# dselivanov/rsparse

Hardware: AMD Instinct MI355X
Metric: als_iterations_per_sec (higher is better)
Workload: dtype f32 (Gram products of rows > 512 / <= 32 non-zeros as 2 x fp16 / 3 x bf16 split terms of the fp32 operands, fp32 accumulate; everything else fp32); 1 GPU; WRMF implicit ALS, CG(3), synthetic 10000000x1000000, 500155883 nnz, rank 128, lambda 0.1; survey_config=3, feedback=implicit, n_items=1000000, nnz=500155883, rank=128, solver=conjugate_gradient, cg_steps=3, parallelism=rows sharded x1, factors replicated

## Files before the change

include/rsparse_wrmf_hip.h:

```cpp
#ifndef RSPARSE_WRMF_HIP_H
#define RSPARSE_WRMF_HIP_H

#include <stddef.h>
#include <stdint.h>

#ifdef __cplusplus
extern "C" {
#endif

#define RSPARSE_HIP_OK 0
#define RSPARSE_HIP_ERR_INVALID 1
#define RSPARSE_HIP_ERR_UNSUPPORTED 2
#define RSPARSE_HIP_ERR_RUNTIME 3
#define RSPARSE_HIP_ERR_NUMERIC 4

#define RSPARSE_SOLVER_CHOLESKY 0
#define RSPARSE_SOLVER_CONJUGATE_GRADIENT 1
#define RSPARSE_SOLVER_NNLS 2

#define RSPARSE_HIP_MAX_RANK 256
#define RSPARSE_HIP_MAX_RANK_F64 128

const char* rsparse_hip_last_error(void);
int rsparse_hip_abi_version(void);
int rsparse_hip_device_count(void);
int rsparse_hip_set_device(int device);


int rsparse_hip_als_implicit_float(int n_rows, int n_cols, const int32_t* col_ptrs,
                                   const int32_t* row_indices, const double* values,
                                   const float* X, float* Y, const float* XtX, int rank,
                                   double lambda, int n_threads, unsigned solver,
                                   unsigned cg_steps, int with_biases, int is_x_bias_last_row,
                                   double global_bias, float* global_bias_base, int global_bias_base_len,
                                   int initialize_bias_base, double* loss_out);

int rsparse_hip_als_implicit_double(int n_rows, int n_cols, const int32_t* col_ptrs,
                                    const int32_t* row_indices, const double* values,
                                    const double* X, double* Y, const double* XtX, int rank,
                                    double lambda, int n_threads, unsigned solver,
                                    unsigned cg_steps, int with_biases, int is_x_bias_last_row,
                                    double global_bias, double* global_bias_base, int global_bias_base_len,
                                    int initialize_bias_base, double* loss_out);

int rsparse_hip_als_explicit_float(int n_rows, int n_cols, const int32_t* col_ptrs,
                                   const int32_t* row_indices, const double* values,
                                   const float* X, float* Y, const float* cnt_X, int rank,
                                   double lambda, unsigned n_threads, unsigned solver,
                                   unsigned cg_steps, int dynamic_lambda, int with_biases,
                                   int is_x_bias_last_row, double* loss_out);

int rsparse_hip_als_explicit_double(int n_rows, int n_cols, const int32_t* col_ptrs,
                                    const int32_t* row_indices, const double* values,
                                    const double* X, double* Y, const double* cnt_X, int rank,
                                    double lambda, unsigned n_threads, unsigned solver,
                                    unsigned cg_steps, int dynamic_lambda, int with_biases,
                                    int is_x_bias_last_row, double* loss_out);

int rsparse_hip_gramian_float(const float* X, int rank, int64_t n, double lambda, float* XtX_out);
int rsparse_hip_gramian_double(const double* X, int rank, int64_t n, double lambda, double* XtX_out);

int rsparse_hip_initialize_biases_float(int n_users, int n_items, const int32_t* csc_p, const int32_t* csc_i,
                                        double* csc_x, const int32_t* csr_p, const int32_t* csr_i, double* csr_x,
                                        float* user_bias, float* item_bias, double lambda, int dynamic_lambda,
                                        int non_negative, int calculate_global_bias, int is_explicit_feedback,
                                        double* global_bias_out);
int rsparse_hip_initialize_biases_double(int n_users, int n_items, const int32_t* csc_p, const int32_t* csc_i,
                                         double* csc_x, const int32_t* csr_p, const int32_t* csr_i, double* csr_x,
                                         double* user_bias, double* item_bias, double lambda, int dynamic_lambda,
                                         int non_negative, int calculate_global_bias, int is_explicit_feedback,
                                         double* global_bias_out);


typedef struct rsparse_hip_csc rsparse_hip_csc;

int rsparse_hip_csc_create_host(int n_rows, int n_cols, const int32_t* col_ptrs,
                                const int32_t* row_indices, const double* values,
                                rsparse_hip_csc** out);
int rsparse_hip_csc_create_device(int n_rows, int n_cols, const int32_t* d_col_ptrs,
                                  const int32_t* d_row_indices, const float* d_values,
                                  rsparse_hip_csc** out);
int rsparse_hip_csc_destroy(rsparse_hip_csc* m);

int rsparse_hip_csc_transpose_device(int n_rows, int n_cols, const int32_t* d_p, const int32_t* d_i,
                                     const float* d_x, int32_t* d_pt, int32_t* d_it, float* d_xt, void* stream);
int rsparse_hip_values_to_float_device(int64_t n, const double* d_src, float* d_dst, void* stream);
int rsparse_hip_csc_freeze_values(rsparse_hip_csc* m, int frozen);

int rsparse_hip_csc_info(const rsparse_hip_csc* m, int64_t info_out[40]);

int rsparse_hip_gramian_device(const float* d_X, int rank, int64_t n, double lambda,
                               float* d_XtX_out, double* d_sumsq_out, void* stream);

int rsparse_hip_gramian_absmax_device(const float* d_X, int rank, int64_t n, double lambda, float* d_XtX_out,
                                      double* d_sumsq_out, float* d_absmax_inout, void* stream);

int rsparse_hip_als_implicit_device(const rsparse_hip_csc* conf, const float* d_X, float* d_Y,
                                    const float* d_XtX, int rank, double lambda, unsigned solver,
                                    unsigned cg_steps, const float* d_absmax, double* d_loss_rows_out, void* stream);

int rsparse_hip_als_explicit_device(const rsparse_hip_csc* conf, const float* d_X, float* d_Y,
                                    int rank, double lambda, unsigned solver, unsigned cg_steps,
                                    int dynamic_lambda, double* d_loss_rows_out, void* stream);

int rsparse_hip_als_implicit_bias_device(const rsparse_hip_csc* conf, const float* d_X, float* d_Y,
                                         const float* d_XtX, int rank, double lambda, unsigned solver,
                                         int is_x_bias_last_row, double* d_loss_rows_out, void* stream);

int rsparse_hip_als_implicit_global_bias_device(const rsparse_hip_csc* conf, const float* d_X, float* d_Y,
                                                const float* d_XtX, int rank, double lambda, unsigned solver,
                                                unsigned cg_steps, int with_biases, int is_x_bias_last_row,
                                                double global_bias, int double_threshold, const float* d_absmax,
                                                double* d_loss_rows_out, void* stream);

int rsparse_hip_initialize_biases_implicit_device(const rsparse_hip_csc* c_ui, const rsparse_hip_csc* c_iu,
                                                  float* d_user_bias, float* d_item_bias, double lambda,
                                                  int non_negative, int calculate_global_bias,
                                                  double* global_bias_out, void* stream);

int rsparse_hip_als_explicit_bias_device(const rsparse_hip_csc* conf, const float* d_X, float* d_Y, int rank,
                                         double lambda, unsigned solver, unsigned cg_steps, int dynamic_lambda,
                                         int is_x_bias_last_row, double* d_loss_rows_out, void* stream);

int rsparse_hip_values_subtract_mean_device(int64_t n, float* d_x, float* d_x_other, double* mean_out, void* stream);

int rsparse_hip_initialize_biases_explicit_device(rsparse_hip_csc* c_ui, rsparse_hip_csc* c_iu, float* d_user_bias,
                                                  float* d_item_bias, double lambda, int dynamic_lambda,
                                                  int non_negative, int calculate_global_bias,
                                                  double* global_bias_out, void* stream);

int rsparse_hip_bias_sweep_explicit_device(const rsparse_hip_csc* conf, const float* d_other_bias, double lambda,
                                           int dynamic_lambda, int non_negative, float* d_out, void* stream);
int rsparse_hip_bias_prep_implicit_device(const rsparse_hip_csc* conf, int n_other, double lambda, double* d_means,
                                          double* d_adj, void* stream);
int rsparse_hip_bias_sweep_implicit_device(const rsparse_hip_csc* conf, const float* d_other_bias, int n_other,
                                           const double* d_other_sum, const double* d_means, const double* d_adj,
                                           int non_negative, double global_bias, float* d_out, void* stream);

int rsparse_hip_weighted_sumsq_device(const float* d_X, int rank, int64_t n, const float* d_w,
                                      double* d_out, void* stream);


#define RSPARSE_HIP_NA_INTEGER INT32_MIN
#define RSPARSE_HIP_MAX_TOPK 256
#define RSPARSE_HIP_MAX_TOPK_LARGE 8192

int rsparse_hip_top_product(const double* x, const double* y, int nr, int nc, int rank, unsigned k,
                            unsigned n_threads, const int32_t* not_recommend_p,
                            const int32_t* not_recommend_j, const int32_t* exclude, int n_exclude,
                            double glob_mean, int32_t* res, double* scores);

int rsparse_hip_top_product_device(const float* d_U, const float* d_V, int n_users, int n_items, int rank,
                                   int k, const int32_t* d_not_recommend_p, const int32_t* d_not_recommend_j,
                                   const int32_t* d_exclude0, int n_exclude, double glob_mean,
                                   int32_t* d_res, float* d_scores, void* stream);

int rsparse_hip_top_product_f64_device(const float* d_U, const float* d_V, const double* d_U64, const double* d_V64,
                                       int n_users, int n_items, int rank, int k, int extra,
                                       const int32_t* d_not_recommend_p, const int32_t* d_not_recommend_j,
                                       const int32_t* d_exclude0, int n_exclude, double glob_mean, int32_t* d_res,
                                       double* d_scores, void* stream);

int rsparse_hip_top_candidates_device(const float* d_U, const float* d_V, int n_users, int n_items, int rank, int k,
                                      const int32_t* d_cand_p, const int32_t* d_cand_j, const int32_t* d_not_recommend_p,
                                      const int32_t* d_not_recommend_j, const int32_t* d_exclude0, int n_exclude,
                                      double glob_mean, int32_t* d_res, double* d_scores, void* stream);
int rsparse_hip_top_candidates_f64_device(const double* d_U, const double* d_V, int n_users, int n_items, int rank, int k,
                                          const int32_t* d_cand_p, const int32_t* d_cand_j, const int32_t* d_not_recommend_p,
                                          const int32_t* d_not_recommend_j, const int32_t* d_exclude0, int n_exclude,
                                          double glob_mean, int32_t* d_res, double* d_scores, void* stream);
int rsparse_hip_top_candidates(const double* x, const double* y, int nr, int nc, int rank, unsigned k, unsigned n_threads,
                               const int32_t* cand_p, const int32_t* cand_j, const int32_t* not_recommend_p,
                               const int32_t* not_recommend_j, const int32_t* exclude, int n_exclude, double glob_mean,
                               int32_t* res, double* scores);


int rsparse_hip_normalize_items_device(const float* d_V, int n_items, int ld, int c0, int c1, float* d_Vn32, double* d_Vn64,
                                       int32_t* d_flags, void* stream);
int rsparse_hip_normalize_items_f64_device(const double* d_V, int n_items, int ld, int c0, int c1, float* d_Vn32,
                                           double* d_Vn64, int32_t* d_flags, void* stream);

int rsparse_hip_similar_items_device(const float* d_Vn32, const double* d_Vn64, int n_items, int r, const int32_t* d_query,
                                     int n_q, int k, int exclude_self, const int32_t* d_exclude0, int n_exclude,
                                     int32_t* d_res, double* d_scores, void* stream);

int rsparse_hip_similar_items(const double* components, int rank, int n_items, int first_row, int n_rows, const int32_t* query,
                              int n_q, int k, int exclude_self, const int32_t* exclude, int n_exclude, int32_t* res,
                              double* scores);


int rsparse_hip_ranking_metrics(const int32_t* predictions, int n_users, int k, const int32_t* actual_p,
                                const int32_t* actual_j, const double* actual_x, double* ap_out, double* ndcg_out);

int rsparse_hip_ranking_metrics_device(const int32_t* d_predictions, int n_users, int k, const int32_t* d_actual_p,
                                       const int32_t* d_actual_j, const double* d_actual_x, double* d_ap_out,
                                       double* d_ndcg_out, void* stream);


#define RSPARSE_HIP_MAX_CUTOFFS 16
int rsparse_hip_hit_metrics_device(const int32_t* d_predictions, int n_users, int k, const int32_t* d_actual_p,
                                   const int32_t* d_actual_j, const int32_t* cutoffs, int n_cutoffs, int32_t* d_hits,
                                   int32_t* d_first, double* d_precision, double* d_recall, double* d_hit, double* d_mrr,
                                   int32_t* d_first_seen, int n_items, void* stream);

int rsparse_hip_hit_metrics(const int32_t* predictions, int n_users, int k, const int32_t* actual_p, const int32_t* actual_j,
                            const int32_t* cutoffs, int n_cutoffs, int32_t* hits, int32_t* first, double* precision,
                            double* recall, double* hit, double* mrr, int32_t* first_seen, int n_items);


int rsparse_hip_list_metrics_device(const int32_t* d_predictions, int n_users, int k, const int32_t* cutoffs, int n_cutoffs,
                                    const int32_t* d_item_count, const int64_t* d_item_info, int n_items, int32_t* d_valid,
                                    int64_t* d_count_sum, int64_t* d_info_sum, double* d_popularity, double* d_novelty,
                                    int32_t* d_exposure, void* stream);

int rsparse_hip_list_metrics(const int32_t* predictions, int n_users, int k, const int32_t* cutoffs, int n_cutoffs,
                             const int32_t* item_count, const int64_t* item_info, int n_items, int32_t* valid,
                             int64_t* count_sum, int64_t* info_sum, double* popularity, double* novelty, int32_t* exposure);

int rsparse_hip_item_inv_norms_device(const float* d_V, int n_items, int ld, int c0, int c1, double* d_inv, void* stream);
int rsparse_hip_item_inv_norms_f64_device(const double* d_V, int n_items, int ld, int c0, int c1, double* d_inv, void* stream);

int rsparse_hip_list_diversity_device(const int32_t* d_predictions, int n_users, int k, const int32_t* cutoffs, int n_cutoffs,
                                      const float* d_V, int n_items, int ld, int c0, int c1, const double* d_inv,
                                      int32_t* d_counted, double* d_diversity, void* stream);
int rsparse_hip_list_diversity_f64_device(const int32_t* d_predictions, int n_users, int k, const int32_t* cutoffs,
                                          int n_cutoffs, const double* d_V, int n_items, int ld, int c0, int c1,
                                          const double* d_inv, int32_t* d_counted, double* d_diversity, void* stream);

int rsparse_hip_list_diversity(const int32_t* predictions, int n_users, int k, const int32_t* cutoffs, int n_cutoffs,
                               const float* V, int n_items, int ld, int c0, int c1, int32_t* counted, double* diversity);
int rsparse_hip_list_diversity_f64(const int32_t* predictions, int n_users, int k, const int32_t* cutoffs, int n_cutoffs,
                                   const double* V, int n_items, int ld, int c0, int c1, int32_t* counted, double* diversity);


int rsparse_hip_mmr_rerank_device(const int32_t* d_lists, const double* d_scores, int n_users, int n_pool, int k, double trade_off,
                                  const float* d_V, int n_items, int ld, int c0, int c1, const double* d_inv, int32_t* d_items,
                                  double* d_scores_out, int32_t* d_positions, double* d_objective, void* stream);
int rsparse_hip_mmr_rerank_f64_device(const int32_t* d_lists, const double* d_scores, int n_users, int n_pool, int k,
                                      double trade_off, const double* d_V, int n_items, int ld, int c0, int c1, const double* d_inv,
                                      int32_t* d_items, double* d_scores_out, int32_t* d_positions, double* d_objective,
                                      void* stream);

// ... 179 lines not shown
```

rsparse_amd/_lib.py:

```python
import ctypes
from pathlib import Path

import os

LIB_PATH = Path(os.environ.get("RSPARSE_HIP_LIB", Path(__file__).resolve().parent / "lib" / "librsparse_wrmf_hip.so"))

OK, ERR_INVALID, ERR_UNSUPPORTED, ERR_RUNTIME, ERR_NUMERIC = 0, 1, 2, 3, 4
SOLVER_CHOLESKY, SOLVER_CG, SOLVER_NNLS = 0, 1, 2
MAX_NEGATIVES = 8192
MAX_CUTOFFS = 16
RANKS_BATCH = 1024

_c_int, _c_uint, _c_dbl, _c_i64, _c_u64 = ctypes.c_int, ctypes.c_uint, ctypes.c_double, ctypes.c_int64, ctypes.c_uint64
_vp = ctypes.c_void_p

SIGNATURES = {
    "rsparse_hip_last_error": (ctypes.c_char_p, []),
    "rsparse_hip_abi_version": (_c_int, []),
    "rsparse_hip_device_count": (_c_int, []),
    "rsparse_hip_set_device": (_c_int, [_c_int]),
    "rsparse_hip_als_implicit_float": (_c_int, [_c_int, _c_int, _vp, _vp, _vp, _vp, _vp, _vp, _c_int, _c_dbl, _c_int,
                                                _c_uint, _c_uint, _c_int, _c_int, _c_dbl, _vp, _c_int, _c_int, _vp]),
    "rsparse_hip_als_implicit_double": (_c_int, [_c_int, _c_int, _vp, _vp, _vp, _vp, _vp, _vp, _c_int, _c_dbl, _c_int,
                                                 _c_uint, _c_uint, _c_int, _c_int, _c_dbl, _vp, _c_int, _c_int, _vp]),
    "rsparse_hip_als_explicit_float": (_c_int, [_c_int, _c_int, _vp, _vp, _vp, _vp, _vp, _vp, _c_int, _c_dbl, _c_uint,
                                                _c_uint, _c_uint, _c_int, _c_int, _c_int, _vp]),
    "rsparse_hip_als_explicit_double": (_c_int, [_c_int, _c_int, _vp, _vp, _vp, _vp, _vp, _vp, _c_int, _c_dbl, _c_uint,
                                                 _c_uint, _c_uint, _c_int, _c_int, _c_int, _vp]),
    "rsparse_hip_gramian_float": (_c_int, [_vp, _c_int, _c_i64, _c_dbl, _vp]),
    "rsparse_hip_gramian_double": (_c_int, [_vp, _c_int, _c_i64, _c_dbl, _vp]),
    "rsparse_hip_csc_create_host": (_c_int, [_c_int, _c_int, _vp, _vp, _vp, ctypes.POINTER(_vp)]),
    "rsparse_hip_csc_create_device": (_c_int, [_c_int, _c_int, _vp, _vp, _vp, ctypes.POINTER(_vp)]),
    "rsparse_hip_gramian_absmax_device": (_c_int, [_vp, _c_int, _c_i64, _c_dbl, _vp, _vp, _vp, _vp]),
    "rsparse_hip_csc_destroy": (_c_int, [_vp]),
    "rsparse_hip_csc_info": (_c_int, [_vp, ctypes.POINTER(_c_i64)]),
    "rsparse_hip_csc_freeze_values": (_c_int, [_vp, _c_int]),
    "rsparse_hip_als_implicit_bias_device": (_c_int, [_vp, _vp, _vp, _vp, _c_int, _c_dbl, _c_uint, _c_int, _vp, _vp]),
    "rsparse_hip_als_implicit_global_bias_device": (_c_int, [_vp, _vp, _vp, _vp, _c_int, _c_dbl, _c_uint, _c_uint, _c_int,
                                                             _c_int, _c_dbl, _c_int, _vp, _vp, _vp]),
    "rsparse_hip_initialize_biases_implicit_device": (_c_int, [_vp, _vp, _vp, _vp, _c_dbl, _c_int, _c_int,
                                                               ctypes.POINTER(_c_dbl), _vp]),
    "rsparse_hip_initialize_biases_float": (_c_int, [_c_int, _c_int, _vp, _vp, _vp, _vp, _vp, _vp, _vp, _vp, _c_dbl, _c_int,
                                                     _c_int, _c_int, _c_int, ctypes.POINTER(_c_dbl)]),
    "rsparse_hip_initialize_biases_double": (_c_int, [_c_int, _c_int, _vp, _vp, _vp, _vp, _vp, _vp, _vp, _vp, _c_dbl, _c_int,
                                                      _c_int, _c_int, _c_int, ctypes.POINTER(_c_dbl)]),
    "rsparse_hip_als_explicit_bias_device": (_c_int, [_vp, _vp, _vp, _c_int, _c_dbl, _c_uint, _c_uint, _c_int, _c_int,
                                                      _vp, _vp]),
    "rsparse_hip_initialize_biases_explicit_device": (_c_int, [_vp, _vp, _vp, _vp, _c_dbl, _c_int, _c_int, _c_int,
                                                               ctypes.POINTER(_c_dbl), _vp]),
    "rsparse_hip_values_subtract_mean_device": (_c_int, [_c_i64, _vp, _vp, ctypes.POINTER(_c_dbl), _vp]),
    "rsparse_hip_bias_sweep_explicit_device": (_c_int, [_vp, _vp, _c_dbl, _c_int, _c_int, _vp, _vp]),
    "rsparse_hip_bias_prep_implicit_device": (_c_int, [_vp, _c_int, _c_dbl, _vp, _vp, _vp]),
    "rsparse_hip_bias_sweep_implicit_device": (_c_int, [_vp, _vp, _c_int, _vp, _vp, _vp, _c_int, _c_dbl, _vp, _vp]),
    "rsparse_hip_bias_sweep_explicit_f64_device": (_c_int, [_vp, _vp, _c_dbl, _c_int, _c_int, _vp, _vp]),
    "rsparse_hip_bias_prep_implicit_f64_device": (_c_int, [_vp, _c_int, _c_dbl, _vp, _vp, _vp]),
    "rsparse_hip_bias_sweep_implicit_f64_device": (_c_int, [_vp, _vp, _c_int, _vp, _vp, _vp, _c_int, _c_dbl, _vp, _vp]),
    "rsparse_hip_csc_transpose_device": (_c_int, [_c_int, _c_int, _vp, _vp, _vp, _vp, _vp, _vp, _vp]),
    "rsparse_hip_values_to_float_device": (_c_int, [_c_i64, _vp, _vp, _vp]),
    "rsparse_hip_gramian_device": (_c_int, [_vp, _c_int, _c_i64, _c_dbl, _vp, _vp, _vp]),
    "rsparse_hip_als_implicit_device": (_c_int, [_vp, _vp, _vp, _vp, _c_int, _c_dbl, _c_uint, _c_uint, _vp, _vp, _vp]),
    "rsparse_hip_als_explicit_device": (_c_int, [_vp, _vp, _vp, _c_int, _c_dbl, _c_uint, _c_uint, _c_int, _vp, _vp]),
    "rsparse_hip_weighted_sumsq_device": (_c_int, [_vp, _c_int, _c_i64, _vp, _vp, _vp]),
    "rsparse_hip_top_product": (_c_int, [_vp, _vp, _c_int, _c_int, _c_int, _c_uint, _c_uint, _vp, _vp, _vp, _c_int, _c_dbl, _vp, _vp]),
    "rsparse_hip_top_product_device": (_c_int, [_vp, _vp, _c_int, _c_int, _c_int, _c_int, _vp, _vp, _vp, _c_int, _c_dbl, _vp, _vp, _vp]),
    "rsparse_hip_top_product_f64_device": (_c_int, [_vp, _vp, _vp, _vp, _c_int, _c_int, _c_int, _c_int, _c_int, _vp, _vp, _vp,
                                                    _c_int, _c_dbl, _vp, _vp, _vp]),
    "rsparse_hip_normalize_items_device": (_c_int, [_vp, _c_int, _c_int, _c_int, _c_int, _vp, _vp, _vp, _vp]),
    "rsparse_hip_normalize_items_f64_device": (_c_int, [_vp, _c_int, _c_int, _c_int, _c_int, _vp, _vp, _vp, _vp]),
    "rsparse_hip_similar_items_device": (_c_int, [_vp, _vp, _c_int, _c_int, _vp, _c_int, _c_int, _c_int, _vp, _c_int, _vp, _vp, _vp]),
    "rsparse_hip_similar_items": (_c_int, [_vp, _c_int, _c_int, _c_int, _c_int, _vp, _c_int, _c_int, _c_int, _vp, _c_int, _vp, _vp]),
    "rsparse_hip_ranking_metrics": (_c_int, [_vp, _c_int, _c_int, _vp, _vp, _vp, _vp, _vp]),
    "rsparse_hip_ranking_metrics_device": (_c_int, [_vp, _c_int, _c_int, _vp, _vp, _vp, _vp, _vp, _vp]),
    "rsparse_hip_hit_metrics_device": (_c_int, [_vp, _c_int, _c_int, _vp, _vp, _vp, _c_int, _vp, _vp, _vp, _vp, _vp, _vp, _vp, _c_int,
                                                _vp]),
    "rsparse_hip_hit_metrics": (_c_int, [_vp, _c_int, _c_int, _vp, _vp, _vp, _c_int, _vp, _vp, _vp, _vp, _vp, _vp, _vp, _c_int]),
    "rsparse_hip_list_metrics_device": (_c_int, [_vp, _c_int, _c_int, _vp, _c_int, _vp, _vp, _c_int, _vp, _vp, _vp, _vp, _vp, _vp, _vp]),
    "rsparse_hip_list_metrics": (_c_int, [_vp, _c_int, _c_int, _vp, _c_int, _vp, _vp, _c_int, _vp, _vp, _vp, _vp, _vp, _vp]),
    "rsparse_hip_item_inv_norms_device": (_c_int, [_vp, _c_int, _c_int, _c_int, _c_int, _vp, _vp]),
    "rsparse_hip_item_inv_norms_f64_device": (_c_int, [_vp, _c_int, _c_int, _c_int, _c_int, _vp, _vp]),
    "rsparse_hip_list_diversity_device": (_c_int, [_vp, _c_int, _c_int, _vp, _c_int, _vp, _c_int, _c_int, _c_int, _c_int, _vp, _vp, _vp,
                                                   _vp]),
    "rsparse_hip_list_diversity_f64_device": (_c_int, [_vp, _c_int, _c_int, _vp, _c_int, _vp, _c_int, _c_int, _c_int, _c_int, _vp, _vp,
                                                       _vp, _vp]),
    "rsparse_hip_list_diversity": (_c_int, [_vp, _c_int, _c_int, _vp, _c_int, _vp, _c_int, _c_int, _c_int, _c_int, _vp, _vp]),
    "rsparse_hip_list_diversity_f64": (_c_int, [_vp, _c_int, _c_int, _vp, _c_int, _vp, _c_int, _c_int, _c_int, _c_int, _vp, _vp]),
    "rsparse_hip_mmr_rerank_device": (_c_int, [_vp, _vp, _c_int, _c_int, _c_int, _c_dbl, _vp, _c_int, _c_int, _c_int, _c_int, _vp, _vp, _vp, _vp, _vp, _vp]),
    "rsparse_hip_mmr_rerank_f64_device": (_c_int, [_vp, _vp, _c_int, _c_int, _c_int, _c_dbl, _vp, _c_int, _c_int, _c_int, _c_int, _vp, _vp, _vp, _vp, _vp, _vp]),
    "rsparse_hip_mmr_rerank": (_c_int, [_vp, _vp, _c_int, _c_int, _c_int, _c_dbl, _vp, _c_int, _c_int, _c_int, _c_int, _vp, _vp, _vp, _vp]),
    "rsparse_hip_mmr_rerank_f64": (_c_int, [_vp, _vp, _c_int, _c_int, _c_int, _c_dbl, _vp, _c_int, _c_int, _c_int, _c_int, _vp, _vp, _vp, _vp]),
    "rsparse_hip_held_out_ranks_device": (_c_int, [_vp, _vp, _c_int, _c_int, _c_int, _vp, _vp, _vp, _c_int, _vp, _vp, _c_int, _vp, _vp,
                                                   _vp, _vp]),
    "rsparse_hip_rank_summary_device": (_c_int, [_c_int, _vp, _vp, _vp, _vp, _vp, _vp, _vp, _vp, _vp, _vp]),
    "rsparse_hip_held_out_ranks": (_c_int, [_vp, _vp, _c_int, _c_int, _c_int, _vp, _vp, _vp, _c_int, _vp, _vp, _vp, _vp, _vp, _vp, _vp,
                                            _vp, _vp, _vp]),
    "rsparse_hip_score_pairs_device": (_c_int, [_vp, _vp, _c_int, _c_int, _c_int, _vp, _vp, _c_dbl, _vp, _vp, _vp, _vp, _vp]),
    "rsparse_hip_score_pairs_f64_device": (_c_int, [_vp, _vp, _c_int, _c_int, _c_int, _vp, _vp, _c_dbl, _vp, _vp, _vp, _vp, _vp]),
    "rsparse_hip_top_candidates_device": (_c_int, [_vp, _vp, _c_int, _c_int, _c_int, _c_int, _vp, _vp, _vp, _vp, _vp, _c_int, _c_dbl, _vp,
                                                   _vp, _vp]),
    "rsparse_hip_top_candidates_f64_device": (_c_int, [_vp, _vp, _c_int, _c_int, _c_int, _c_int, _vp, _vp, _vp, _vp, _vp, _c_int, _c_dbl,
                                                       _vp, _vp, _vp]),
    "rsparse_hip_top_candidates": (_c_int, [_vp, _vp, _c_int, _c_int, _c_int, _c_uint, _c_uint, _vp, _vp, _vp, _vp, _vp, _c_int, _c_dbl,
                                            _vp, _vp]),
    "rsparse_hip_explain_device": (_c_int, [_vp, _c_int, _c_int, _vp, _c_dbl, _c_dbl, _c_int, _vp, _vp, _vp, _vp, _vp, _vp, _vp, _vp,
                                            _vp, _vp, _vp]),
    "rsparse_hip_explain_f64_device": (_c_int, [_vp, _c_int, _c_int, _vp, _c_dbl, _c_dbl, _c_int, _vp, _vp, _vp, _vp, _vp, _vp, _vp,
                                                _vp, _vp, _vp, _vp]),
    "rsparse_hip_init_factors_device": (_c_int, [_c_u64, _c_int, _c_i64, _c_int, _c_int, _c_i64, _c_dbl, _c_int, _c_int, _vp, _vp]),
    "rsparse_hip_init_factors_f64_device": (_c_int, [_c_u64, _c_int, _c_i64, _c_int, _c_int, _c_i64, _c_dbl, _c_int, _c_int, _vp,
                                                     _vp]),
    "rsparse_hip_sample_negatives_device": (_c_int, [_c_u64, _c_i64, _c_int, _c_int, _c_int, _vp, _vp, _vp, _vp, _vp, _vp, _c_i64, _vp]),
    "rsparse_hip_sample_negatives": (_c_int, [_c_u64, _c_i64, _c_int, _c_int, _c_int, _vp, _vp, _vp, _vp, _vp, _vp, _c_i64]),
    "rsparse_hip_weights_prefix_device": (_c_int, [_vp, _c_int, _vp, _vp]),
    "rsparse_hip_sample_negatives_weighted_device": (_c_int, [_c_u64, _c_i64, _c_int, _c_int, _c_int, _vp, _vp, _vp, _vp, _vp, _vp, _vp, _c_i64, _vp, _vp]),
    "rsparse_hip_sample_negatives_weighted": (_c_int, [_c_u64, _c_i64, _c_int, _c_int, _c_int, _vp, _vp, _vp, _vp, _vp, _vp, _vp, _c_i64, _vp]),
    "rsparse_hip_split_rows_device": (_c_int, [_c_u64, _c_i64, _c_int, _c_int, _c_u64, _c_int, _c_int, _vp, _vp, _vp, _c_int, _vp, _vp, _vp, _vp, _vp, _vp, _vp, _c_i64, _c_i64, _vp]),
    "rsparse_hip_split_rows": (_c_int, [_c_u64, _c_i64, _c_int, _c_int, _c_u64, _c_int, _c_int, _vp, _vp, _vp, _c_int, _vp, _vp, _vp, _vp, _vp, _vp, _vp, _c_i64, _c_i64]),
    "rsparse_hip_confidence_moments_device": (_c_int, [_c_int, _c_i64, _vp, _vp, _c_int, _vp, _vp, _vp]),
    "rsparse_hip_confidence_table_device": (_c_int, [_c_int, _c_int, _vp, _vp, _vp, _c_dbl, _c_dbl, _c_dbl, _vp, _vp]),
    "rsparse_hip_confidence_apply_device": (_c_int, [_c_int, _c_int, _c_i64, _vp, _vp, _vp, _vp, _vp, _c_int, _c_int, _c_dbl, _c_dbl, _vp, _c_int, _vp]),
    "rsparse_hip_confidence": (_c_int, [_c_int, _c_int, _c_int, _vp, _vp, _vp, _c_dbl, _c_dbl, _c_int, _c_int, _vp]),
    "rsparse_hip_events_to_csr_device": (_c_int, [_c_i64, _c_int, _c_int, _vp, _vp, _vp, _vp, _c_int, _c_dbl, _c_dbl, _c_int, _vp, _vp, _vp, _vp, _vp,
                                                  _c_i64, ctypes.POINTER(_c_i64), _vp]),
    "rsparse_hip_events_to_csr": (_c_int, [_c_i64, _c_int, _c_int, _vp, _vp, _vp, _vp, _c_int, _c_dbl, _c_dbl, _c_int, _vp, _vp, _vp, _vp, _vp,
                                           _c_i64, ctypes.POINTER(_c_i64)]),
    "rsparse_hip_sparse_approximation": (_c_int, [_c_int, _c_int, _vp, _vp, _c_int, _vp, _vp, _c_int, _vp]),
    "rsparse_hip_csc_f64_create_device": (_c_int, [_c_int, _c_int, _vp, _vp, _vp, ctypes.POINTER(_vp)]),
    "rsparse_hip_csc_f64_destroy": (_c_int, [_vp]),
    "rsparse_hip_gramian_f64_device": (_c_int, [_vp, _c_int, _c_i64, _c_dbl, _vp, _vp, _vp]),
    "rsparse_hip_als_f64_device": (_c_int, [_vp, _c_int, _vp, _vp, _vp, _c_int, _c_dbl, _c_uint, _c_uint, _c_int, _c_int,
                                            _c_int, _c_dbl, _vp, _vp]),
    "rsparse_hip_initialize_biases_f64_device": (_c_int, [_vp, _vp, _vp, _vp, _c_dbl, _c_int, _c_int, _c_int, _c_int,
                                                          ctypes.POINTER(_c_dbl), _vp]),
    "rsparse_hip_values_subtract_mean_f64_device": (_c_int, [_c_i64, _vp, _vp, ctypes.POINTER(_c_dbl), _vp]),
    "rsparse_hip_weighted_sumsq_f64_device": (_c_int, [_vp, _c_int, _c_i64, _vp, _vp, _vp]),
    "rsparse_hip_profile_enable": (_c_int, [_c_int]),
    "rsparse_hip_set_launch_mode": (_c_int, [_c_int]),
    "rsparse_hip_set_f64_long_rows": (_c_int, [_c_int, _c_int]),
    "rsparse_hip_profile_last": (_c_int, [ctypes.POINTER(_c_dbl)]),
    "rsparse_hip_profile_last_names": (_c_int, [ctypes.c_char_p, _c_int]),
    "rsparse_hip_take_numeric_failures": (_c_int, [ctypes.POINTER(_c_i64), ctypes.POINTER(_c_i64)]),
    "rsparse_hip_ctx_create": (_c_int, [_c_int, _vp, _c_int, ctypes.POINTER(_vp)]),
    "rsparse_hip_ctx_destroy": (_c_int, [_vp]),
    "rsparse_hip_ctx_set_matrix": (_c_int, [_vp, _c_int, _c_int, _vp, _vp, _vp, _vp, _vp, _vp, _c_int, _c_int]),
    "rsparse_hip_ctx_set_factors": (_c_int, [_vp, _c_int, _vp, _vp]),
    "rsparse_hip_ctx_get_factors": (_c_int, [_vp, _vp, _vp]),
    "rsparse_hip_ctx_half_iteration": (_c_int, [_vp, _c_int, _c_int, _c_dbl, _c_uint, _c_uint, _c_int, ctypes.POINTER(_c_dbl)]),
    "rsparse_hip_ctx_take_numeric_failures": (_c_int, [_vp, ctypes.POINTER(_c_i64), ctypes.POINTER(_c_i64)]),
    "rsparse_hip_ctx_info": (_c_int, [_vp, ctypes.POINTER(_c_i64), ctypes.POINTER(_c_dbl)]),
}


class RsparseHipError(RuntimeError):
    def __init__(self, code, msg):
        super().__init__("librsparse_wrmf_hip: [%d] %s" % (code, msg))
        self.code = code


class UnsupportedOnDevice(RsparseHipError, NotImplementedError):
    """RSPARSE_HIP_ERR_UNSUPPORTED: the reference-side shim would keep its CPU path here."""


_lib = None


def load():
    global _lib
    if _lib is None:
        if not LIB_PATH.exists():
            raise RuntimeError(
                "%s not found -- the HIP extension is required (no CPU fallback). "
                "Build it with `python -m rsparse_amd.build`." % LIB_PATH)
        try:
            import torch
            torch.cuda.is_available()
        except ImportError:
            pass
        lib = ctypes.CDLL(str(LIB_PATH))
        for name, (res, args) in SIGNATURES.items():
            f = getattr(lib, name)
            f.restype, f.argtypes = res, args
        _lib = lib
    return _lib


def check(code):
    if code == OK:
        return
    msg = load().rsparse_hip_last_error().decode("utf-8", "replace")
# ... 4 lines not shown
```

rsparse_amd/build.py:

```python
import subprocess
import sys
import time
from concurrent.futures import ThreadPoolExecutor
from pathlib import Path

PKG = Path(__file__).resolve().parent
CSRC = PKG / "csrc"
SRC = [CSRC / n for n in ("wrmf_kernels.hip", "wrmf_cgq.hip", "wrmf_cgp.hip", "wrmf_ne.hip", "wrmf_chol.hip", "wrmf_chol_wave.hip", "wrmf_chol_mf.hip", "wrmf_cg_mf.hip", "wrmf_chol_lr.hip",
                          "wrmf_topk.hip", "wrmf_topk_large.hip", "wrmf_similar.hip", "wrmf_metrics.hip", "wrmf_hits.hip", "wrmf_lists.hip", "wrmf_diversity.hip", "wrmf_mmr.hip", "wrmf_ranks.hip", "wrmf_score.hip", "wrmf_candidates.hip", "wrmf_sample.hip", "wrmf_sample_weighted.hip", "wrmf_split.hip", "wrmf_confidence.hip", "wrmf_events.hip", "wrmf_explain.hip", "wrmf_init.hip", "wrmf_ingest.hip", "wrmf_nnls.hip", "wrmf_bias.hip", "wrmf_lu.hip",
                          "wrmf_f64.hip", "wrmf_wide.hip", "wrmf_wide_cg.hip", "wrmf_ctx_kernels.hip", "wrmf_schedule.cpp", "wrmf_capi.cpp", "wrmf_f64_capi.cpp", "wrmf_ctx.cpp")]
HEADERS = [CSRC / "wrmf_chol_mf.attrs.csv", CSRC / "wrmf_mf.h", CSRC / "wrmf_internal.h", CSRC / "wrmf_capi_common.h", CSRC / "wrmf_schedule.h", CSRC / "wrmf_device.h", CSRC / "wrmf_sample_team.h", CSRC / "wrmf_wave.h", CSRC / "wrmf_ldlt.h", CSRC / "wrmf_f64.h", PKG.parent / "include" / "rsparse_wrmf_hip.h"]
DEPS = SRC + HEADERS
OUT = PKG / "lib" / "librsparse_wrmf_hip.so"
FLAGS = ["--offload-arch=gfx950", "-O3", "-std=c++17", "-fPIC"]


EXTRA_FLAGS = {n: ["-mllvm", "-forceattrs-csv-path=" + str(CSRC / "wrmf_chol_mf.attrs.csv"), "-fno-slp-vectorize"] for n in ("wrmf_chol_mf.hip", "wrmf_cg_mf.hip")}
AUDITED = {"wrmf_chol_mf.hip", "wrmf_cg_mf.hip"}
REG_LIMIT = {"wrmf_cg_mf.hip": 512}
NO_SPILL = {"wrmf_cgq.hip": ("14als_cgq_kernelILi128ELi24ELi4ELi4E",),
            "wrmf_cgp.hip": ("14als_cgp_kernelILb0ELb1ELi16ELb1E",),
            "wrmf_explain.hip": ("14explain_kernelIfLi128E",),
            "wrmf_sample.hip": ("13sample_kernelILi64E", "13sample_kernelILi256E"),
            "wrmf_sample_weighted.hip": ("22sample_weighted_kernelILi64E", "22sample_weighted_kernelILi256E"),
            "wrmf_hits.hip": ("18hit_metrics_kernelILb0E", "18hit_metrics_kernelILb1E"),
            "wrmf_lists.hip": ("19list_metrics_kernelILb0E", "19list_metrics_kernelILb1E"),
            "wrmf_diversity.hip": ("21list_diversity_kernelI", "21item_inv_norms_kernelI"),
            "wrmf_mmr.hip": ("10mmr_kernelI",),
            "wrmf_confidence.hip": ("conf_moments_kernel", "conf_moments_finish_kernel", "conf_table_kernel", "conf_apply_kernel"),
            "wrmf_events.hip": ("events_pack_kernel", "events_now_kernel", "events_heads_kernel", "events_reduce_kernel",
                                "events_long_chunks_kernel", "events_long_finish_kernel"),
            "wrmf_cg_mf.hip": ("rsparse_hip_als_cg_mf_implicit", "rsparse_hip_als_cg_mf_implicit_any"),
            "wrmf_split.hip": ("split_count_wave_kernel", "split_count_team_kernel", "split_write_wave_kernel", "split_write_team_kernel")}
RESOURCE_FLAG = "-Rpass-analysis=kernel-resource-usage"


def resource_violations(remarks, patterns, limit=256):
    import re
    rows, cur = [], None
    for line in remarks.splitlines():
        m = re.search(r"remark:\s+(.*?) \[-Rpass", line)
        if not m:
            continue
        t = m.group(1).strip()
        if t.startswith("Function Name:"):
            cur = {"name": t.split(":", 1)[1].strip()}
            rows.append(cur)
        elif ":" in t and cur is not None:
            k, v = t.rsplit(":", 1)
            cur[k.strip()] = v.strip()
    bad = []
    for pat in patterns:
        hit = [r for r in rows if pat in r["name"]]
        if not hit:
            bad.append((pat, "no such kernel in the compilation"))
        for r in hit:
            regs = int(r.get("VGPRs", "0")) + int(r.get("AGPRs", "0"))
            for key in ("VGPRs Spill", "ScratchSize [bytes/lane]"):
                if int(r.get(key, "0")):
                    bad.append((r["name"], "%s = %s" % (key, r[key])))
            if regs > limit:
                bad.append((r["name"], "%d vector registers" % regs))
    return bad


def audit_listing(src, extra, obj):
    sys.path.insert(0, str(PKG.parent / "tools" / "dbg"))
    import acc_audit
    lst = obj.with_suffix(".s")

    def listing(flags, floor):
        cmd = ["hipcc", *FLAGS, *flags, "-S", "--cuda-device-only", str(src), "-o", str(lst)]
        r = subprocess.run(cmd, stdout=subprocess.PIPE, stderr=subprocess.PIPE, text=True)
        if r.returncode != 0:
            raise RuntimeError("hipcc -S failed on %s:\n%s" % (src.name, r.stderr[-3000:]))
        acc, flight, _ = acc_audit.audit(str(lst), quiet=True, acc_floor=floor)
        return acc, flight, lst.read_text()
    acc, flight, text = listing(extra, 0)
    import re
    nfree = re.findall(r"\.amdhsa_kernel (\w+)[\s\S]*?\.amdhsa_next_free_vgpr (\d+)", text)
    limit = REG_LIMIT.get(src.name, 256)
    two_waves = bool(nfree) and all(int(v) <= limit for name, v in nfree if "_any" not in name)
    if acc == 0 and flight == 0 and two_waves:
        return
    print("  %s: audit of the two-waves-per-SIMD build failed (accumulator-file %d, in-flight %d, layout ok %s): rebuilding with -DMF_SAFE"
          % (src.name, acc, flight, two_waves), flush=True)
    safe = ["-DMF_SAFE"]
    cmd = ["hipcc", *FLAGS, *safe, "-c", str(src), "-o", str(obj)]
    r = subprocess.run(cmd, stdout=subprocess.PIPE, stderr=subprocess.PIPE, text=True)
    if r.returncode != 0:
        raise RuntimeError("hipcc failed on %s (MF_SAFE):\n%s" % (src.name, r.stderr[-3000:]))
    acc, flight, text = listing(safe, 96)
    if acc or flight:
        raise RuntimeError("%s: the MF_SAFE build fails the audit too (accumulator-file %d, in-flight %d)" % (src.name, acc, flight))


def build(force=False, verbose=False, out=None):
    out = Path(out) if out else OUT
    out.parent.mkdir(exist_ok=True)
    objdir = OUT.parent / "obj"
    objdir.mkdir(parents=True, exist_ok=True)
    src = [s for s in SRC if s.exists()]
    hdr_m = max(h.stat().st_mtime for h in HEADERS)
    todo, objs = [], []
    for s in src:
        o = objdir / (s.stem + ".o")
        objs.append(o)
        if force or not o.exists() or o.stat().st_mtime < max(s.stat().st_mtime, hdr_m):
            todo.append((s, o))
    if not todo and out.exists() and all(out.stat().st_mtime >= o.stat().st_mtime for o in objs):
        return out

    def compile_one(so):
        s, o = so
        t0 = time.time()
        extra = EXTRA_FLAGS.get(s.name, [])
        guard = NO_SPILL.get(s.name)
        cmd = ["hipcc", *FLAGS, *extra, *([RESOURCE_FLAG] if guard else []), "-c", str(s), "-o", str(o)]
        r = subprocess.run(cmd, stdout=subprocess.PIPE, stderr=subprocess.PIPE, text=True)
        if r.returncode != 0:
            raise RuntimeError("hipcc failed on %s:\n%s" % (s.name, r.stderr[-6000:]))
        if guard:
            bad = resource_violations(r.stderr, guard, REG_LIMIT.get(s.name, 256))
            if bad:
                o.unlink()
                raise RuntimeError("%s: kernels that must not spill do:\n%s" % (s.name, "\n".join("  %s: %s" % b for b in bad)))
        if s.name in AUDITED:
            audit_listing(s, extra, o)
        if verbose:
            print("  %-20s %.1f s" % (s.name, time.time() - t0), flush=True)

    with ThreadPoolExecutor(max_workers=8) as ex:
        list(ex.map(compile_one, todo))
    cmd = ["hipcc", "--offload-arch=gfx950", "-fPIC", "-shared", *map(str, objs), "-ldl", "-lpthread", "-o", str(out)]
    subprocess.check_call(cmd)
    return out


if __name__ == "__main__":
    argv = sys.argv[1:]
    outp = argv[argv.index("--out") + 1] if "--out" in argv else None
    t0 = time.time()
    print(build(force="--force" in argv, verbose=True, out=outp), "%.1f s" % (time.time() - t0))
```

rsparse_amd/csrc/wrmf_capi.cpp:

```cpp
#include "../../include/rsparse_wrmf_hip.h"

#include <cxxabi.h>

#include <algorithm>
#include <cfloat>
#include <cmath>
#include <cstdlib>
#include <cstring>
#include <string>
#include <vector>

#include "wrmf_capi_common.h"

using namespace rsparse_hip;

struct rsparse_hip_csc {
  DevCSC d;
  int device = 0;
  std::vector<void*> owned;
};

namespace {
thread_local std::string g_err;
}

int rsparse_hip::capi_fail(int code, const std::string& msg) {
  g_err = msg;
  return code;
}
int rsparse_hip::capi_hip_fail(hipError_t e, const char* what) {
  return fail(RSPARSE_HIP_ERR_RUNTIME, std::string(what) + ": " + hipGetErrorString(e));
}

namespace {

using CscGuard = HandleGuard<rsparse_hip_csc, rsparse_hip_csc_destroy>;

struct Workspace {
  GrowBufBase* all = nullptr;
  GrowBuf<float> gram{all};
  GrowBuf<double> partials{all};
  GrowBuf<double> scalars{all};
  GrowBuf<int> fails{all};
  GrowBuf<unsigned> ne_stats{all};
  GrowBuf<float> lr_M{all};
  GrowBuf<float> ne_seg_scratch{all};
  GrowBuf<int> ne_seg_flags{all};
  GrowBuf<float> zero_row{all};
  GrowBuf<float> tscr{all};
  GrowBuf<float> bias_buf{all};
  GrowBuf<float> gb_r0{all};
  GrowBuf<int32_t> gb_slot{all};
  GrowBuf<float> wide_m2{all};
  GrowBuf<float> wide_lu{all};
  GrowBuf<int> met_buf{all};
  GrowBuf<char> sim_buf{all};
  GrowBuf<double> score_buf{all};
  GrowBuf<float> mf_G{all};
  GrowBuf<float> pad_buf{all};
  int device = -1;

  int ensure_device() {
    int dev = 0;
    HIP_TRY(hipGetDevice(&dev));
    if (dev != device) {
      GrowBufBase::release_all(all);
      device = dev;
    }
    if (!scalars) {
      HIP_TRY(scalars.ensure(16));
      HIP_TRY(hipMemset(scalars, 0, 16 * sizeof(double)));
    }
    if (!fails) {
      HIP_TRY(fails.ensure((size_t)(4 + kFailCap)));
      HIP_TRY(hipMemset(fails, 0, 4 * sizeof(int)));
    }
    if (!ne_stats) {
      HIP_TRY(ne_stats.ensure(4));
      HIP_TRY(hipMemset(ne_stats, 0, 4 * sizeof(unsigned)));
    }
    if (!zero_row) {
      HIP_TRY(zero_row.ensure(256));
      HIP_TRY(hipMemset(zero_row, 0, 256 * sizeof(float)));
    }
    return RSPARSE_HIP_OK;
  }
  int ensure_partials(size_t slots) {
    HIP_TRY(partials.ensure(std::max<size_t>(slots, 1024) + kSumStageBlocks));
    return RSPARSE_HIP_OK;
  }
  size_t partial_slots() const { return partials.cap - kSumStageBlocks; }
};
thread_local Workspace g_ws;

int sum_scratch(SumScratch& w) {
  int rc = g_ws.ensure_device();
  if (rc) return rc;
  if ((rc = g_ws.ensure_partials(1024))) return rc;
  w = {g_ws.partials, g_ws.scalars};
  return RSPARSE_HIP_OK;
}

struct Profiler {
  bool on = false;
  bool have = false;
  int nseg = 0;
  hipEvent_t ev[10] = {nullptr, nullptr, nullptr, nullptr, nullptr, nullptr, nullptr, nullptr, nullptr, nullptr};
  const void* kern[10] = {nullptr, nullptr, nullptr, nullptr, nullptr, nullptr, nullptr, nullptr, nullptr, nullptr};
  hipEvent_t* begin() {
    have = false;
    if (!on) return nullptr;
    for (auto& e : ev)
      if (!e && hipEventCreate(&e) != hipSuccess) return nullptr;
    for (auto& k : kern) k = nullptr;
    return ev;
  }
};
thread_local Profiler g_prof;

template <class T>
int upload(rsparse_hip_csc& m, const std::vector<T>& v, const T** out) {
  *out = nullptr;
  if (v.empty()) return RSPARSE_HIP_OK;
  void* p = nullptr;
  HIP_TRY(hipMalloc(&p, v.size() * sizeof(T)));
  m.owned.push_back(p);
  HIP_TRY(hipMemcpy(p, v.data(), v.size() * sizeof(T), hipMemcpyHostToDevice));
  *out = static_cast<const T*>(p);
  return RSPARSE_HIP_OK;
}

int upload_cut(rsparse_hip_csc& m, const NeCut& cut, NeListSet& L) {
  L = NeListSet();
  L.entries = (int)cut.items.size();
  L.nseg = cut.nseg();
  L.nsplit = (int)cut.split_rows.size();
  if (int rc = upload(m, cut.segs, &L.segs)) return rc;
  if (int rc = upload(m, cut.split_rows, &L.split_rows)) return rc;
  return upload(m, cut.split_ptr, &L.split_ptr);
}
int upload_deal(rsparse_hip_csc& m, const NeDeal& deal, NeListSet& L) {
  L.wg = deal.wg();
  if (int rc = upload(m, deal.rows, &L.rows)) return rc;
  return upload(m, deal.ptr, &L.ptr);
}

int build_schedule(rsparse_hip_csc& m, const int32_t* host_col_ptrs) {
  DevCSC& d = m.d;
  int cus = 256;
  HIP_TRY(hipDeviceGetAttribute(&cus, hipDeviceAttributeMultiprocessorCount, m.device));
  d.q_cfg = cgq_default_cfg();
  SchedulePlan plan;
  if (!plan_schedule(host_col_ptrs, d.n_cols, cus, [](int len) { return cgq_bucket_of(len, cgq_default_cfg()); }, plan))
    return fail(RSPARSE_HIP_ERR_INVALID, "col_ptrs is not non-decreasing");
  d.max_len = plan.max_len; d.nnz_long = plan.nnz_long; d.n_empty = plan.n_empty;
  d.short_max = kTileNnz; d.n_long = plan.n_long;
  for (int b = 0; b < 7; b++) d.q_off[b] = plan.off[b];
  for (int b = 0; b < 6; b++) d.q_nnz[b] = plan.nnz[b];
  d.q_pair_first = plan.pair_first; d.q_team4_first = plan.team4_first;
  d.q_team4_wide_first = plan.team4_wide_first;
  d.q_gt32 = plan.gt32; d.q_gt48 = plan.gt48; d.q_lr_first = plan.lr_first; d.q_n_lr = plan.n_lr;
  d.q_n_chol_long = plan.n_chol_long; d.q_n_nec = plan.n_nec;
  int rc;
  if ((rc = upload(m, plan.order, &d.q_order))) return rc;
  if ((rc = upload(m, plan.stream_off, &d.q_stream_off))) return rc;
  if ((rc = upload_cut(m, plan.cut, d.q_ne))) return rc;
  d.q_ne1 = d.q_ne;
  if ((rc = upload_deal(m, plan.fine, d.q_ne))) return rc;
  if ((rc = upload_deal(m, plan.coarse, d.q_ne1))) return rc;
  if (plan.nec_is_ne) {
    d.q_nec = d.q_ne;
  } else {
    if ((rc = upload_cut(m, plan.cut_nec, d.q_nec))) return rc;
    if ((rc = upload_deal(m, plan.nec, d.q_nec))) return rc;
  }
  return RSPARSE_HIP_OK;
}

bool use_cgq(int rank, const void* X, const void* Y) {
  return rank % 4 == 0 && ((reinterpret_cast<uintptr_t>(X) | reinterpret_cast<uintptr_t>(Y)) & 15) == 0;
}

int check_common(int n_rows, int n_cols, const void* col_ptrs, const void* X, const void* Y, int rank) {
  if (n_rows < 0 || n_cols < 0) return fail(RSPARSE_HIP_ERR_INVALID, "negative matrix dimension");
  if (!col_ptrs) return fail(RSPARSE_HIP_ERR_INVALID, "col_ptrs is NULL");
  if (!X || !Y) return fail(RSPARSE_HIP_ERR_INVALID, "X or Y is NULL");
  if (rank <= 0) return fail(RSPARSE_HIP_ERR_INVALID, "rank must be positive");
  if (rank > RSPARSE_HIP_MAX_RANK)
    return fail(RSPARSE_HIP_ERR_UNSUPPORTED, "rank > 256 is not on the device path");
  return RSPARSE_HIP_OK;
}

thread_local int64_t g_fail_carry[2] = {0, 0};

bool has_global_bias(double global_bias, bool dbl = false) {
  return global_bias >= std::sqrt(dbl ? DBL_EPSILON : (double)FLT_EPSILON);
}

bool zero_padding_is_neutral(bool implicit, unsigned solver, double lambda) {
  return implicit || solver != RSPARSE_SOLVER_CHOLESKY || lambda != 0.0;
}

int check_variant(unsigned solver, int with_biases, double global_bias, bool implicit = true) {
  if (solver > RSPARSE_SOLVER_NNLS) return fail(RSPARSE_HIP_ERR_INVALID, "unknown solver code");
  if (with_biases && implicit && solver == RSPARSE_SOLVER_CONJUGATE_GRADIENT)
    return fail(RSPARSE_HIP_ERR_UNSUPPORTED, "with_user_item_bias + conjugate_gradient with implicit feedback is not on the device path");
  (void)global_bias;
  return RSPARSE_HIP_OK;
}

struct BiasTerms {
  const float* rhs_vals;
  const float* loss_tgt;
  const float* rhs_init;
  float tgt_const = 1.f;
  float gbias = 0.f;
};

hipError_t take_value_stats(const DevCSC& d, const float* d_X, int64_t nx, hipStream_t s, const float* d_absmax) {
  if (d.vals_frozen && !d.vstats && hipMalloc(&d.vstats, 2 * sizeof(unsigned)) != hipSuccess) d.vstats = nullptr;
  if (d.vals_frozen && d.vstats && d.vstats_valid && d.vstats_stream == s)
    return launch_ne_stats(d_X, nx, d.vals, d.nnz, g_ws.ne_stats, s, d_absmax, d.vstats, nullptr);
  hipError_t e = launch_ne_stats(d_X, nx, d.vals, d.nnz, g_ws.ne_stats, s, d_absmax, nullptr,
                                 (d.vals_frozen && d.vstats) ? d.vstats : nullptr);
  if (e == hipSuccess && d.vals_frozen && d.vstats) { d.vstats_valid = true; d.vstats_stream = s; }
  return e;
}

int run_half_iteration(const rsparse_hip_csc* conf, bool implicit, const float* d_X, float* d_Y,
                       const float* d_XtX, int rank, double lambda, unsigned solver, unsigned cg_steps,
                       int dynamic_lambda, double* d_loss_rows_out, hipStream_t s, const BiasTerms* bias = nullptr,
                       const float* d_absmax = nullptr) {
  if (!conf) return fail(RSPARSE_HIP_ERR_INVALID, "conf is NULL");
  if (!d_X || !d_Y) return fail(RSPARSE_HIP_ERR_INVALID, "X or Y is NULL");
  if (implicit && !d_XtX) return fail(RSPARSE_HIP_ERR_INVALID, "XtX is NULL");
  if (rank <= 0) return fail(RSPARSE_HIP_ERR_INVALID, "rank must be positive");
  if (rank > RSPARSE_HIP_MAX_RANK) return fail(RSPARSE_HIP_ERR_UNSUPPORTED, "rank > 256 is not on the device path");
  int rc = check_variant(solver, 0, 0.0);
  if (rc) return rc;
  if ((rc = g_ws.ensure_device())) return rc;
  const DevCSC& d = conf->d;
  const bool pad_to_128 = solver == RSPARSE_SOLVER_CHOLESKY && !bias && rank > 64 && rank < 128 && zero_padding_is_neutral(implicit, solver, lambda);
  const bool pad_to_64 = solver == RSPARSE_SOLVER_CHOLESKY && !bias && rank < 64 && zero_padding_is_neutral(implicit, solver, lambda);
  if (((rank % 4 != 0 && rank < 128) || pad_to_128 || pad_to_64) && zero_padding_is_neutral(implicit, solver, lambda)) {
    const int kp = pad_to_128 ? 128 : (pad_to_64 ? 64 : ((rank + 3) & ~3));
    const size_t nx = (size_t)d.n_rows * kp, ny = (size_t)d.n_cols * kp, ng = (size_t)kp * kp;
    HIP_TRY(g_ws.pad_buf.ensure(nx + ny + ng + 256 + 16));
    float* Xp = g_ws.pad_buf;
    float* Yp = Xp + nx;
    float* Gp = Yp + ny;
    float* rp = Gp + ng;
    hipError_t e;
    if ((e = launch_pad_rows(d_X, rank, 0, rank, kp, d.n_rows, Xp, s)) != hipSuccess) return hip_fail(e, "launch_pad_rows");
    if ((e = launch_pad_rows(d_Y, rank, 0, rank, kp, d.n_cols, Yp, s)) != hipSuccess) return hip_fail(e, "launch_pad_rows");
    if (implicit && (e = launch_pad_gramian(d_XtX, rank, kp, Gp, s)) != hipSuccess) return hip_fail(e, "launch_pad_gramian");
    BiasTerms bp;
    if (bias) {
      bp = *bias;
      if (bias->rhs_init) {
        if ((e = launch_pad_rows(bias->rhs_init, rank, 0, rank, kp, 1, rp, s)) != hipSuccess) return hip_fail(e, "launch_pad_rows");
        bp.rhs_init = rp;
      }
    }
    rc = run_half_iteration(conf, implicit, Xp, Yp, implicit ? Gp : nullptr, kp, lambda, solver, cg_steps, dynamic_lambda,
                            d_loss_rows_out, s, bias ? &bp : nullptr, d_absmax);
    if (rc) return rc;
    if (d.n_cols > 0)
      HIP_TRY(hipMemcpy2DAsync(d_Y, (size_t)rank * 4, Yp, (size_t)kp * 4, (size_t)rank * 4, (size_t)d.n_cols,
                               hipMemcpyDeviceToDevice, s));
    return RSPARSE_HIP_OK;
  }
  if (wide_supported(rank)) {
    double* outw = d_loss_rows_out ? d_loss_rows_out : g_ws.scalars;
    if (d.n_cols == 0) {
      HIP_TRY(hipMemsetAsync(outw, 0, sizeof(double), s));
      return RSPARSE_HIP_OK;
    }
    const int grid = wide_als_grid(d.n_cols);
    const int grid_w = wide_cg_wave_grid(d.n_cols) + wide_cg_team_grid(d.n_cols);
    if ((rc = g_ws.ensure_partials((size_t)grid + (size_t)grid_w))) return rc;
    HIP_TRY(g_ws.wide_m2.ensure(solver == RSPARSE_SOLVER_NNLS ? (size_t)grid * wide_m2_floats_per_wg(rank) : 0));
    HIP_TRY(g_ws.wide_lu.ensure(solver == RSPARSE_SOLVER_CHOLESKY ? (size_t)grid * rank * rank : 0));
    AlsArgs a{};
    a.col_ptrs = d.col_ptrs; a.row_idx = d.row_idx; a.vals = d.vals;
    a.X = d_X; a.Y = d_Y; a.XtX = implicit ? d_XtX : nullptr;
    a.n_cols = d.n_cols; a.k = rank; a.cg_steps = (int)cg_steps;
    a.lambda = (float)lambda; a.lambda_loss = lambda; a.dynamic_lambda = dynamic_lambda ? 1 : 0;
    a.loss_partials = g_ws.partials; a.fail_counter = g_ws.fails;
    a.rhs_vals = bias ? bias->rhs_vals : nullptr;
    a.loss_tgt = bias ? bias->loss_tgt : nullptr;
    a.rhs_init = bias ? bias->rhs_init : nullptr;
    a.loss_tgt_const = bias ? bias->tgt_const : 1.f;
    a.gbias = (solver == RSPARSE_SOLVER_CONJUGATE_GRADIENT && implicit && bias) ? bias->gbias : 0.f;
    const bool wave_cg = wide_cg_wave_supported(a, solver) && (d.q_order || d.max_len <= kWideCgMaxLen);
    hipError_t we = wave_cg ? launch_wide_cg_wave(a, implicit, kWideCgMaxLen, d.max_len > kWideCgMaxLen ? d.q_order : nullptr, 0, s)
                            : launch_als_wide(a, implicit, solver, g_ws.wide_m2, g_ws.wide_lu, s);
    if (we != hipSuccess) return hip_fail(we, wave_cg ? "launch_wide_cg_wave" : "launch_als_wide");
    if ((we = launch_sum_partials(g_ws.partials, wave_cg ? (size_t)grid_w : (size_t)grid, outw, s, g_ws.partials + g_ws.partial_slots())) != hipSuccess)
      return hip_fail(we, "launch_sum_partials");
    return RSPARSE_HIP_OK;
  }
  const bool cg = solver == RSPARSE_SOLVER_CONJUGATE_GRADIENT;
  const bool cgq = cg && use_cgq(rank, d_X, d_Y);
  QSchedule qs;
  qs.order = d.q_order;
  qs.cfg = d.q_cfg;
  qs.pair_first = d.q_pair_first;
  for (int b = 0; b < 7; b++) qs.off[b] = d.q_off[b];
  qs.team4_first = (implicit && bias && bias->gbias != 0.f) ? d.q_off[2] : d.q_team4_first;
  qs.team4_wide_first = (implicit && bias && bias->gbias != 0.f) ? d.q_off[2] : d.q_team4_wide_first;
  qs.pair_wide = cgp_wide_supported(rank, implicit, implicit && bias && bias->gbias != 0.f);
  qs.pair_quad = cgp_quad_supported(rank, implicit, implicit && bias && bias->gbias != 0.f);
  const bool cg_mf = cgq && implicit && !bias && cg_mf_supported(rank, implicit) && d.q_order && d.q_off[1] > d.q_n_nec;
  if (cg_mf) {
    qs.mf_rows = d.q_order + d.q_n_nec;
    qs.mf_n = d.q_off[1] - d.q_n_nec;
  }
  const bool chol_mf = chol_mf_supported(rank) && !cg && solver == RSPARSE_SOLVER_CHOLESKY && !bias && d.q_order && ne_supported(rank) &&
                       use_cgq(rank, d_X, d_Y) && d.q_lr_first > d.q_off[1];
  const int mf_first = d.q_off[1];
  const int n_mf = chol_mf ? d.q_lr_first - mf_first : 0;
  const bool nec_lists = padded_rank(rank) > 64 && d.q_nec.wg > 0 && !chol_mf;
  const bool ne_chol = !cg && solver == RSPARSE_SOLVER_CHOLESKY && !bias && (nec_lists || d.q_ne.wg > 0 || chol_mf) &&
                       ne_supported(rank) && use_cgq(rank, d_X, d_Y);
  qs.ne = (cg_mf || (ne_chol && nec_lists)) ? d.q_nec : ((implicit && padded_rank(rank) == 128) ? d.q_ne : d.q_ne1);
  const size_t chol_base = chol2_loss_slots(d.n_cols);
  const size_t slots = cgq ? cgq_loss_slots(qs, rank, implicit) : (cg ? cg_loss_slots(d.n_cols, d.n_long)
                                   : (solver == RSPARSE_SOLVER_NNLS ? chol_loss_slots(d.n_cols)
                                      : chol_base + (ne_chol ? (size_t)(qs.ne.entries + qs.ne.nsplit) : 0) +
                                            (size_t)(chol_mf ? chol_mf_loss_slots(n_mf, implicit) : 0) + (size_t)kLuGrid));
  if ((rc = g_ws.ensure_partials(slots))) return rc;
  double* out = d_loss_rows_out ? d_loss_rows_out : g_ws.scalars;
  if (d.n_cols == 0) {
    HIP_TRY(hipMemsetAsync(out, 0, sizeof(double), s));
    return RSPARSE_HIP_OK;
  }
  AlsArgs a;
  a.col_ptrs = d.col_ptrs; a.row_idx = d.row_idx; a.vals = d.vals;
  a.X = d_X; a.Y = d_Y; a.XtX = implicit ? d_XtX : nullptr;
  a.long_rows = d.n_long ? d.q_order : nullptr; a.n_long = d.n_long; a.n_cols = d.n_cols;
  a.chol_long_rows = d.q_order; a.n_chol_long = d.q_order ? d.q_n_chol_long : 0;
  a.chol_list = nullptr; a.chol_first = 0; a.chol_n_main = 0; a.chol_empty_first = 0;
  a.lr_rows = nullptr; a.n_lr = 0; a.lr_flags = nullptr; a.lr_M = nullptr; a.lr_n_gt32 = a.lr_n_gt16 = a.lr_n_gt48 = -1; a.lrx = 0;
  a.nnls_order = solver == RSPARSE_SOLVER_NNLS ? d.q_order : nullptr;
  a.nnls_lhs = nullptr;
  if (solver == RSPARSE_SOLVER_NNLS && padded_rank(rank) == 128) {
    HIP_TRY(g_ws.wide_m2.ensure(chol_loss_slots(d.n_cols) * (size_t)128 * 128));
    a.nnls_lhs = g_ws.wide_m2;
  }
  a.k = rank; a.cg_steps = (int)cg_steps;
  a.lambda = (float)lambda; a.lambda_loss = lambda; a.dynamic_lambda = dynamic_lambda ? 1 : 0;
  a.loss_partials = g_ws.partials; a.fail_counter = g_ws.fails; a.zero_row = g_ws.zero_row;
  a.fail_rows = g_ws.fails + 4; a.fail_cap = kFailCap;
  a.rhs_vals = bias ? bias->rhs_vals : nullptr;
  a.loss_tgt = bias ? bias->loss_tgt : nullptr;
  a.rhs_init = bias ? bias->rhs_init : nullptr;
  a.loss_tgt_const = bias ? bias->tgt_const : 1.f;
  const bool gb_cg = cg && implicit && bias && bias->gbias != 0.f;
  a.gbias = gb_cg ? bias->gbias : 0.f;
  a.ne_r0 = nullptr; a.ne_r0_slot = nullptr;
  a.tscr = nullptr; a.stream_off = d.q_stream_off; a.stream_nnz = d.q_nnz[0];
  a.ne_stats = nullptr; a.wave_stats = nullptr; a.mf_XtX = nullptr;
  a.ne_segs = nullptr; a.ne_seg_scratch = nullptr; a.ne_seg_flags = nullptr;
  a.ne_chol = ne_chol ? 1 : 0;
  a.ne_chol_min = nec_lists ? kCgMfMax : kNeMinLen;
  if (d.q_order && solver == RSPARSE_SOLVER_CHOLESKY) {
    const int first = chol_mf ? d.q_lr_first : (ne_chol ? (nec_lists ? d.q_n_nec : d.q_off[1]) : d.q_n_chol_long);
    a.chol_list = d.q_order;
    a.chol_first = first;
    a.chol_n_main = std::max(0, d.q_lr_first - first);
    a.chol_empty_first = d.q_lr_first + d.q_n_lr;
  }
  if ((cgq || ne_chol) && qs.ne.nseg > 0 && ne_supported(rank)) {
    HIP_TRY(g_ws.ne_seg_scratch.ensure((size_t)qs.ne.nseg * (size_t)kNeSegFloats));
    HIP_TRY(g_ws.ne_seg_flags.ensure((size_t)qs.ne.nseg));
    a.ne_segs = qs.ne.segs; a.ne_seg_scratch = g_ws.ne_seg_scratch; a.ne_seg_flags = g_ws.ne_seg_flags;
  }
  bool stats_taken = false;
  auto want_stats = [&]() -> int {
    if (stats_taken) return RSPARSE_HIP_OK;
    hipError_t se = take_value_stats(d, d_X, (int64_t)d.n_rows * rank, s, d_absmax);
    if (se != hipSuccess) return hip_fail(se, "launch_ne_stats");
    stats_taken = true;
    return RSPARSE_HIP_OK;
  };
  if (chol_mf) {
    if ((rc = want_stats())) return rc;
    a.wave_stats = g_ws.ne_stats;
    if (implicit) {
      a.ne_stats = g_ws.ne_stats;
      a.mf_XtX = d_XtX;
      if (rank != 128) {
        HIP_TRY(g_ws.mf_G.ensure((size_t)128 * 128));
        hipError_t pe = launch_pad_gramian(d_XtX, rank, 128, g_ws.mf_G, s);
        if (pe != hipSuccess) return hip_fail(pe, "launch_pad_gramian");
        a.mf_XtX = g_ws.mf_G;
      }
    }
  }
  if (!a.ne_stats && (cgq || ne_chol) && implicit && (qs.ne.wg > 0 || qs.mf_n > 0) && ne_supported(rank) && (!bias || gb_cg)) {
    if ((rc = want_stats())) return rc;
    a.ne_stats = g_ws.ne_stats;
    if (gb_cg && cgq) {
      const int n_ne = d.q_off[1];
      HIP_TRY(g_ws.gb_r0.ensure((size_t)n_ne * rank));
      HIP_TRY(g_ws.gb_slot.ensure((size_t)d.n_cols));
      hipError_t ge = launch_gb_row_terms(a, d.q_order, n_ne, g_ws.gb_r0, g_ws.gb_slot, s);
      if (ge != hipSuccess) return hip_fail(ge, "launch_gb_row_terms");
      a.ne_r0 = g_ws.gb_r0; a.ne_r0_slot = g_ws.gb_slot;
    }
  }
  if (cgq && !ne_supported(rank) && d.q_stream_off && d.q_nnz[0] > 0 && cg_steps >= 1 && cg_steps <= 4) {
    HIP_TRY(g_ws.tscr.ensure((size_t)(cg_steps + 1) * (size_t)d.q_nnz[0]));
    a.tscr = g_ws.tscr;
  }
  if (!cg && solver == RSPARSE_SOLVER_CHOLESKY && d.q_order && d.q_n_lr > 0 && chol_lr_supported(a, implicit)) {
    HIP_TRY(g_ws.lr_M.ensure((size_t)3 * 128 * 128));
    if ((rc = want_stats())) return rc;
    a.lr_rows = d.q_order + d.q_lr_first; a.n_lr = d.q_n_lr; a.lr_flags = g_ws.ne_stats + 2; a.lr_M = g_ws.lr_M;
    a.lr_n_gt32 = d.q_gt32 - d.q_lr_first; a.lr_n_gt16 = d.q_pair_first - d.q_lr_first;
    a.lr_n_gt48 = d.q_gt48 - d.q_lr_first;
  }
  const bool chol = !cg && solver == RSPARSE_SOLVER_CHOLESKY;
  if (chol && d.q_order && d.q_n_lr > 0 && chol_lrx_supported(a, implicit)) {
    if ((rc = want_stats())) return rc;
    a.wave_stats = g_ws.ne_stats;
    a.lr_rows = d.q_order + d.q_lr_first; a.n_lr = d.q_n_lr; a.lrx = 1;
    a.lr_n_gt32 = d.q_gt32 - d.q_lr_first; a.lr_n_gt16 = d.q_pair_first - d.q_lr_first;
    a.lr_n_gt48 = d.q_gt48 - d.q_lr_first;
  }
  if (chol && chol_wave_supported(rank) && padded_rank(rank) == 64) {
    if ((rc = want_stats())) return rc;
    a.wave_stats = g_ws.ne_stats;
  }
  if (chol) {
    hipError_t fe = launch_fail_roll(g_ws.fails, s);
    if (fe != hipSuccess) return hip_fail(fe, "launch_fail_roll");
  }
  hipEvent_t* ev = g_prof.begin();
  if (chol && ev) HIP_TRY(hipEventRecord(ev[0], s));
  if (ne_chol && qs.ne.wg > 0 && mf_first != 0) {
    hipError_t ne = launch_als_ne(a, qs, implicit, g_ws.partials + chol_base, s, ev);
    if (ne != hipSuccess) return hip_fail(ne, "launch_als_ne");
  }
  hipError_t e = cgq ? launch_als_cgq(a, qs, implicit, s, ev)
                     : (cg ? launch_als_cg(a, implicit, s, ev)
                           : (solver == RSPARSE_SOLVER_NNLS
                                  ? launch_als_nnls(a, implicit, s, ev)
                                  : launch_als_chol2(a, implicit, s, ev ? ev + 1 : nullptr)));
  if (e != hipSuccess) return hip_fail(e, cgq ? "launch_als_cgq" : (cg ? "launch_als_cg" : "launch_als_chol"));
  if (chol_mf) {
    const size_t mf_base = chol_base + (size_t)(qs.ne.entries + qs.ne.nsplit);
    hipError_t me = launch_als_chol_mf(a, implicit, d.q_order + mf_first, n_mf, (int)mf_base, s, ev ? ev + 3 : nullptr);
    if (me != hipSuccess) return hip_fail(me, "launch_als_chol_mf");
  }
  if (chol && ev) HIP_TRY(hipEventRecord(ev[4], s));
  if (chol) {
    if ((e = launch_als_lu_fallback(a, implicit, slots - (size_t)kLuGrid, s)) != hipSuccess)
      return hip_fail(e, "launch_als_lu_fallback");
  }
  e = launch_sum_partials(g_ws.partials, slots, out, s, g_ws.partials + g_ws.partial_slots());
  if (e != hipSuccess) return hip_fail(e, "launch_sum_partials");
  if (ev) {
    const int last = cgq ? 7 : (chol ? 5 : 3);
    HIP_TRY(hipEventRecord(ev[last], s));
// ... 169 lines not shown

extern "C" {

const char* rsparse_hip_last_error(void) { return g_err.c_str(); }
int rsparse_hip_abi_version(void) { return 6; }

int rsparse_hip_device_count(void) {
  int n = 0;
  if (hipGetDeviceCount(&n) != hipSuccess) {
    (void)hipGetLastError();
    return 0;
  }
  return n;
}

int rsparse_hip_set_device(int device) {
  HIP_TRY(hipSetDevice(device));
  return RSPARSE_HIP_OK;
}

int rsparse_hip_csc_create_host(int n_rows, int n_cols, const int32_t* col_ptrs, const int32_t* row_indices,
                                const double* values, rsparse_hip_csc** out) {
  if (!out) return fail(RSPARSE_HIP_ERR_INVALID, "out is NULL");
  *out = nullptr;
  if (n_rows < 0 || n_cols < 0) return fail(RSPARSE_HIP_ERR_INVALID, "negative matrix dimension");
  if (!col_ptrs) return fail(RSPARSE_HIP_ERR_INVALID, "col_ptrs is NULL");
  const int64_t nnz = (int64_t)col_ptrs[n_cols] - col_ptrs[0];
  if (col_ptrs[0] != 0 || nnz < 0) return fail(RSPARSE_HIP_ERR_INVALID, "col_ptrs must start at 0 and be non-decreasing");
  if (nnz > 0 && (!row_indices || !values)) return fail(RSPARSE_HIP_ERR_INVALID, "row_indices or values is NULL");
  for (int64_t e = 0; e < nnz; e++)
    if (row_indices[e] < 0 || row_indices[e] >= n_rows)
      return fail(RSPARSE_HIP_ERR_INVALID, "row index out of range");
  rsparse_hip_csc* m = new rsparse_hip_csc();
  CscGuard guard{m};
  if (hipGetDevice(&m->device) != hipSuccess) return fail(RSPARSE_HIP_ERR_RUNTIME, "no HIP device");
  DevCSC& d = m->d;
  d.n_rows = n_rows; d.n_cols = n_cols; d.nnz = nnz;
  int32_t *dp = nullptr, *di = nullptr;
  float* dv = nullptr;
  HIP_TRY(hipMalloc(&dp, ((size_t)n_cols + 1) * 4));
  m->owned.push_back(dp);
  d.col_ptrs = dp;
  HIP_TRY(hipMalloc(&di, (size_t)std::max<int64_t>(nnz, 4) * 4));
  m->owned.push_back(di);
  d.row_idx = di;
  HIP_TRY(hipMalloc(&dv, (size_t)std::max<int64_t>(nnz, 4) * 4));
  m->owned.push_back(dv);
  d.vals = dv;
  HIP_TRY(hipMemcpy(dp, col_ptrs, ((size_t)n_cols + 1) * 4, hipMemcpyHostToDevice));
  if (nnz) {
    HIP_TRY(hipMemcpy(di, row_indices, (size_t)nnz * 4, hipMemcpyHostToDevice));
    std::vector<float> v32(values, values + nnz);
    HIP_TRY(hipMemcpy(dv, v32.data(), (size_t)nnz * 4, hipMemcpyHostToDevice));
  }
  if (int rc = build_schedule(*m, col_ptrs)) return rc;
  guard.c = nullptr;
  *out = m;
  return RSPARSE_HIP_OK;
}

int rsparse_hip_csc_create_device(int n_rows, int n_cols, const int32_t* d_col_ptrs, const int32_t* d_row_indices,
                                  const float* d_values, rsparse_hip_csc** out) {
  if (!out) return fail(RSPARSE_HIP_ERR_INVALID, "out is NULL");
  *out = nullptr;
  if (n_rows < 0 || n_cols < 0) return fail(RSPARSE_HIP_ERR_INVALID, "negative matrix dimension");
  if (!d_col_ptrs) return fail(RSPARSE_HIP_ERR_INVALID, "col_ptrs is NULL");
  std::vector<int32_t> hp((size_t)n_cols + 1);
  HIP_TRY(hipMemcpy(hp.data(), d_col_ptrs, hp.size() * 4, hipMemcpyDeviceToHost));
  if (hp[0] != 0) return fail(RSPARSE_HIP_ERR_INVALID, "col_ptrs must start at 0");
  const int64_t nnz = hp[n_cols];
  if (nnz > 0 && (!d_row_indices || !d_values)) return fail(RSPARSE_HIP_ERR_INVALID, "row_indices or values is NULL");
  if (nnz < 0) return fail(RSPARSE_HIP_ERR_INVALID, "col_ptrs must be non-decreasing");
  for (int c = 0; c < n_cols; c++)
    if (hp[(size_t)c + 1] < hp[(size_t)c]) return fail(RSPARSE_HIP_ERR_INVALID, "col_ptrs must be non-decreasing");
  {
    int bad = 0;
    HIP_TRY(check_row_indices_device(d_row_indices, nnz, n_rows, nullptr, &bad));
    if (bad) return fail(RSPARSE_HIP_ERR_INVALID, "row index out of range");
  }
  rsparse_hip_csc* m = new rsparse_hip_csc();
  CscGuard guard{m};
  if (hipGetDevice(&m->device) != hipSuccess) return fail(RSPARSE_HIP_ERR_RUNTIME, "no HIP device");
  DevCSC& d = m->d;
  d.n_rows = n_rows; d.n_cols = n_cols; d.nnz = nnz;
  d.col_ptrs = d_col_ptrs; d.row_idx = d_row_indices; d.vals = d_values;
  if (int rc = build_schedule(*m, hp.data())) return rc;
  guard.c = nullptr;
  *out = m;
  return RSPARSE_HIP_OK;
}

int rsparse_hip_csc_transpose_device(int n_rows, int n_cols, const int32_t* d_p, const int32_t* d_i, const float* d_x,
                                     int32_t* d_pt, int32_t* d_it, float* d_xt, void* stream) {
  if (n_rows < 0 || n_cols < 0) return fail(RSPARSE_HIP_ERR_INVALID, "negative matrix dimension");
  if (!d_p || !d_pt) return fail(RSPARSE_HIP_ERR_INVALID, "col_ptrs (input or output) is NULL");
  hipStream_t s = static_cast<hipStream_t>(stream);
  int32_t ends[2] = {0, 0};
  HIP_TRY(hipMemcpyAsync(&ends[0], d_p, 4, hipMemcpyDeviceToHost, s));
  HIP_TRY(hipMemcpyAsync(&ends[1], d_p + n_cols, 4, hipMemcpyDeviceToHost, s));
  HIP_TRY(hipStreamSynchronize(s));
  const int64_t nnz = (int64_t)ends[1] - ends[0];
  if (ends[0] != 0 || nnz < 0) return fail(RSPARSE_HIP_ERR_INVALID, "col_ptrs must start at 0 and be non-decreasing");
  if (nnz > 0 && (!d_i || !d_x || !d_it || !d_xt)) return fail(RSPARSE_HIP_ERR_INVALID, "index or value array is NULL");
  int bad = 0;
  hipError_t e = transpose_csc_device(n_rows, n_cols, nnz, d_p, d_i, d_x, d_pt, d_it, d_xt, s, &bad);
  if (bad) return fail(RSPARSE_HIP_ERR_INVALID, "row index out of range");
  if (e != hipSuccess) return hip_fail(e, "transpose_csc_device");
  return RSPARSE_HIP_OK;
}

int rsparse_hip_values_to_float_device(int64_t n, const double* d_src, float* d_dst, void* stream) {
  if (n < 0) return fail(RSPARSE_HIP_ERR_INVALID, "negative length");
  if (n > 0 && (!d_src || !d_dst)) return fail(RSPARSE_HIP_ERR_INVALID, "NULL array");
  if (n == 0) return RSPARSE_HIP_OK;
  hipError_t e = launch_f64_to_f32(d_src, d_dst, (size_t)n, static_cast<hipStream_t>(stream));
  if (e != hipSuccess) return hip_fail(e, "launch_f64_to_f32");
  return RSPARSE_HIP_OK;
}

int rsparse_hip_csc_destroy(rsparse_hip_csc* m) {
  if (!m) return RSPARSE_HIP_OK;
  for (void* p : m->owned) (void)hipFree(p);
  if (m->d.vstats) (void)hipFree(m->d.vstats);
  delete m;
  return RSPARSE_HIP_OK;
}

int rsparse_hip_csc_freeze_values(rsparse_hip_csc* m, int frozen) {
  if (!m) return fail(RSPARSE_HIP_ERR_INVALID, "NULL handle");
  m->d.vals_frozen = frozen != 0;
  m->d.vstats_valid = false;
  return RSPARSE_HIP_OK;
}

int rsparse_hip_csc_info(const rsparse_hip_csc* m, int64_t info_out[40]) {
  if (!m || !info_out) return fail(RSPARSE_HIP_ERR_INVALID, "NULL argument");
  for (int b = 0; b < 40; b++) info_out[b] = 0;
  for (int b = 0; b < 6; b++) {
    info_out[8 + b] = m->d.q_off[b + 1] - m->d.q_off[b];
    info_out[14 + b] = m->d.q_nnz[b];
  }
  info_out[20] = m->d.q_cfg;
  info_out[21] = m->d.q_ne.nseg;
  for (int b = 0; b < 6; b++) {
    info_out[22 + b] = cgq_bucket_wpr(m->d.q_cfg, b);
    info_out[28 + b] = cgq_bucket_capq(m->d.q_cfg, b);
    info_out[34 + b] = cgq_bucket_waves(m->d.q_cfg, b) * (cgq_bucket_stream(m->d.q_cfg, b) ? -1 : 1);
  }
  info_out[0] = m->d.n_rows; info_out[1] = m->d.n_cols; info_out[2] = m->d.nnz;
  info_out[3] = m->d.n_long; info_out[4] = m->d.max_len; info_out[5] = m->d.nnz_long;
  info_out[6] = m->d.n_empty; info_out[7] = m->d.short_max;
  return RSPARSE_HIP_OK;
}

int rsparse_hip_set_launch_mode(int mode) {
  if (mode < 0 || mode > 2) return fail(RSPARSE_HIP_ERR_INVALID, "launch mode must be 0, 1 or 2");
  cgq_set_launch_mode(mode);
  return RSPARSE_HIP_OK;
}

int rsparse_hip_profile_enable(int on) {
  g_prof.on = on != 0;
  g_prof.have = false;
  return RSPARSE_HIP_OK;
}

int rsparse_hip_profile_last_names(char* buf, int cap) {
  if (!buf || cap <= 0) return fail(RSPARSE_HIP_ERR_INVALID, "buf is NULL or empty");
  buf[0] = 0;
  if (!g_prof.on || !g_prof.have) return fail(RSPARSE_HIP_ERR_INVALID, "no profiled call to report");
  std::string out;
  for (int i = 0; i < g_prof.nseg; i++) {
    if (i) out += '\n';
    if (!g_prof.kern[i]) continue;
    const char* mangled = hipKernelNameRefByPtr(g_prof.kern[i], nullptr);
    if (!mangled) continue;
    int st = 0;
    char* dem = abi::__cxa_demangle(mangled, nullptr, nullptr, &st);
    if (st != 0 || !dem) {
      std::string alt(mangled);
      for (size_t p2; (p2 = alt.find("DF16_")) != std::string::npos;) alt.replace(p2, 5, "Dh");
      std::free(dem);
      dem = abi::__cxa_demangle(alt.c_str(), nullptr, nullptr, &st);
    }
    out += (st == 0 && dem) ? dem : mangled;
    std::free(dem);
  }
  if ((int)out.size() + 1 > cap) return fail(RSPARSE_HIP_ERR_INVALID, "buffer too small for the kernel names");
  std::memcpy(buf, out.c_str(), out.size() + 1);
  return RSPARSE_HIP_OK;
}

int rsparse_hip_profile_last(double ms_out[8]) {
  if (!ms_out) return fail(RSPARSE_HIP_ERR_INVALID, "ms_out is NULL");
  for (int i = 0; i < 8; i++) ms_out[i] = 0.0;
  if (!g_prof.on || !g_prof.have) return fail(RSPARSE_HIP_ERR_INVALID, "no profiled call to report");
  HIP_TRY(hipEventSynchronize(g_prof.ev[g_prof.nseg]));
  for (int i = 0; i < g_prof.nseg; i++) {
    float ms = 0.f;
    HIP_TRY(hipEventElapsedTime(&ms, g_prof.ev[i], g_prof.ev[i + 1]));
    ms_out[i] = ms;
  }
  return RSPARSE_HIP_OK;
}

int rsparse_hip_gramian_device(const float* d_X, int rank, int64_t n, double lambda, float* d_XtX_out,
                               double* d_sumsq_out, void* stream) {
  return rsparse_hip_gramian_absmax_device(d_X, rank, n, lambda, d_XtX_out, d_sumsq_out, nullptr, stream);
}

int rsparse_hip_gramian_absmax_device(const float* d_X, int rank, int64_t n, double lambda, float* d_XtX_out,
                                      double* d_sumsq_out, float* d_absmax_inout, void* stream) {
  if ((!d_X && n != 0) || !d_XtX_out) return fail(RSPARSE_HIP_ERR_INVALID, "X or XtX_out is NULL");
  if (rank <= 0 || n < 0) return fail(RSPARSE_HIP_ERR_INVALID, "rank must be positive and n non-negative");
  if (rank > RSPARSE_HIP_MAX_RANK) return fail(RSPARSE_HIP_ERR_UNSUPPORTED, "rank > 256 is not on the device path");
  int rc = g_ws.ensure_device();
  if (rc) return rc;
  if (wide_supported(rank)) {
    HIP_TRY(g_ws.gram.ensure(wide_gramian_scratch_floats(rank)));
    hipError_t we = launch_gramian_wide(d_X, rank, n, (float)lambda, d_XtX_out, d_sumsq_out, g_ws.gram, (hipStream_t)stream);
    if (we != hipSuccess) return hip_fail(we, "launch_gramian_wide");
    return RSPARSE_HIP_OK;
  }
  HIP_TRY(g_ws.gram.ensure(gramian_scratch_floats(rank, n)));
  const float ridge = (float)lambda;
  hipEvent_t* ev = g_prof.begin();
  hipError_t e = launch_gramian(d_X, rank, n, ridge, d_XtX_out, d_sumsq_out, g_ws.gram, (hipStream_t)stream, ev,
                                reinterpret_cast<unsigned*>(d_absmax_inout));
  if (e != hipSuccess) return hip_fail(e, "launch_gramian");
  if (ev) {
    g_prof.have = true;
    g_prof.nseg = 2;
  }
  return RSPARSE_HIP_OK;
}

int rsparse_hip_gramian_float(const float* X, int rank, int64_t n, double lambda, float* XtX_out) {
  return gramian_host(X, rank, n, XtX_out, [&](const float* dX, float* dG) {
    return rsparse_hip_gramian_device(dX, rank, n, lambda, dG, nullptr, nullptr);
  });
}

int rsparse_hip_als_implicit_device(const rsparse_hip_csc* conf, const float* d_X, float* d_Y, const float* d_XtX,
                                    int rank, double lambda, unsigned solver, unsigned cg_steps,
                                    const float* d_absmax, double* d_loss_rows_out, void* stream) {
  return run_half_iteration(conf, true, d_X, d_Y, d_XtX, rank, lambda, solver, cg_steps, 0, d_loss_rows_out,
                            (hipStream_t)stream, nullptr, d_absmax);
}

int rsparse_hip_als_explicit_device(const rsparse_hip_csc* conf, const float* d_X, float* d_Y, int rank,
                                    double lambda, unsigned solver, unsigned cg_steps, int dynamic_lambda,
                                    double* d_loss_rows_out, void* stream) {
  return run_half_iteration(conf, false, d_X, d_Y, nullptr, rank, lambda, solver, cg_steps, dynamic_lambda,
                            d_loss_rows_out, (hipStream_t)stream);
}

int rsparse_hip_als_implicit_bias_device(const rsparse_hip_csc* conf, const float* d_X, float* d_Y, const float* d_XtX,
                                         int rank, double lambda, unsigned solver, int is_x_bias_last_row,
                                         double* d_loss_rows_out, void* stream) {
  int rc = check_variant(solver, 1, 0.0, true);
  if (rc) return rc;
  return run_half_iteration_implicit_biased(conf, d_X, d_Y, d_XtX, rank, lambda, solver, is_x_bias_last_row,
                                            d_loss_rows_out, (hipStream_t)stream);
}

int rsparse_hip_als_implicit_global_bias_device(const rsparse_hip_csc* conf, const float* d_X, float* d_Y,
                                                const float* d_XtX, int rank, double lambda, unsigned solver,
                                                unsigned cg_steps, int with_biases, int is_x_bias_last_row,
                                                double global_bias, int double_threshold, const float* d_absmax,
                                                double* d_loss_rows_out, void* stream) {
  int rc = check_variant(solver, with_biases, global_bias, true);
  if (rc) return rc;
  if (with_biases)
    return run_half_iteration_implicit_biased(conf, d_X, d_Y, d_XtX, rank, lambda, solver, is_x_bias_last_row,
                                              d_loss_rows_out, (hipStream_t)stream, global_bias, double_threshold != 0);
  if (!has_global_bias(global_bias, double_threshold != 0))
    return run_half_iteration(conf, true, d_X, d_Y, d_XtX, rank, lambda, solver, cg_steps, 0, d_loss_rows_out,
                              (hipStream_t)stream, nullptr, d_absmax);
  return run_half_iteration_implicit_global(conf, d_X, d_Y, d_XtX, rank, lambda, solver, cg_steps, global_bias, nullptr,
                                            nullptr, d_loss_rows_out, (hipStream_t)stream, d_absmax);
}

int rsparse_hip_initialize_biases_implicit_device(const rsparse_hip_csc* c_ui, const rsparse_hip_csc* c_iu,
                                                  float* d_user_bias, float* d_item_bias, double lambda,
                                                  int non_negative, int calculate_global_bias,
                                                  double* global_bias_out, void* stream) {
  if (!c_ui || !c_iu || !d_user_bias || !d_item_bias) return fail(RSPARSE_HIP_ERR_INVALID, "NULL matrix or bias vector");
  const CscView<float> a(c_ui->d), b(c_iu->d);
  if (a.n_rows != b.n_cols || a.n_cols != b.n_rows || a.nnz != b.nnz)
    return fail(RSPARSE_HIP_ERR_INVALID, "the two matrices are not transposes of each other");
  SumScratch w;
  if (int rc = sum_scratch(w)) return rc;
  return initialize_biases_implicit(a, b, d_user_bias, d_item_bias, lambda, non_negative, calculate_global_bias, w,
                                    (hipStream_t)stream, global_bias_out);
}

int rsparse_hip_bias_sweep_explicit_device(const rsparse_hip_csc* conf, const float* d_other_bias, double lambda,
                                           int dynamic_lambda, int non_negative, float* d_out, void* stream) {
  if (!conf || !d_other_bias || !d_out) return fail(RSPARSE_HIP_ERR_INVALID, "NULL matrix or bias vector");
  return bias_sweep_explicit(CscView<float>(conf->d), d_other_bias, (float)lambda, dynamic_lambda, non_negative, d_out,
                             (hipStream_t)stream);
}

int rsparse_hip_bias_prep_implicit_device(const rsparse_hip_csc* conf, int n_other, double lambda, double* d_means,
                                          double* d_adj, void* stream) {
  if (!conf || !d_means || !d_adj) return fail(RSPARSE_HIP_ERR_INVALID, "NULL matrix or output");
// ... 1513 lines not shown
```

rsparse_amd/csrc/wrmf_cgp.hip:

```cpp
#include "wrmf_internal.h"
#include "wrmf_device.h"

namespace rsparse_hip {
namespace {

using namespace dev;

constexpr int kPairMaxSweeps = 4;

template <int NQ, bool QUAD = false>
struct PairSmem {
  static constexpr int KP = 128, ps = KP + 8, os = QUAD ? KP + 8 : KP + 4;
  static constexpr int cols = QUAD ? 16 : 8;
  static constexpr int pcs = QUAD ? 2 * ps : ps;
  static constexpr size_t gfrag = NQ == 16 ? (size_t)4 * 16 * 1024 : 0;
  static constexpr size_t nxt = NQ == 16 ? (size_t)4 * 2 * 2 * 64 * 4 : 0;
  static constexpr size_t pub = (size_t)2 * cols * ps * 2, out = (size_t)cols * os * 4;
  static_assert(!QUAD || (pub == out && (size_t)pcs * 2 == (size_t)os * 4), "QUAD: one column, one stretch of LDS");
  static constexpr size_t bytes = gfrag + (QUAD ? pub : pub + out) + (size_t)4 * 8 * NQ * 4 + nxt + 16;
};
static_assert(PairSmem<16>::bytes <= 81920 && PairSmem<16, true>::bytes <= 81920, "two workgroups per CU");

template <bool GB, bool KFULL = false, int NQ = 8, bool QUAD = false>
__global__ __launch_bounds__(256, 2) void als_cgp_kernel(AlsArgs a, const int32_t* __restrict__ rows, int n_rows, int iters,
                                                        size_t loss_slot0) {
  constexpr int KP = 128, RPN = 8, VW = 4, NV = 2;
  static_assert(NQ == 8 || (NQ == 16 && KFULL && !GB), "the 32-slot kernel: rank 128, no global bias");
  static_assert(!QUAD || NQ == 16, "four rows per wave: 16 slots per group, G in LDS");
  constexpr bool GREG = NQ == 8;
  constexpr int RW = QUAD ? 4 : 2, GL = 64 / RW;
  constexpr int SS = QUAD ? 1 : 2;
  using SM = PairSmem<NQ, QUAD>;
  extern __shared__ __attribute__((aligned(16))) char smem[];
  char* sGf = smem + (size_t)(threadIdx.x >> 6) * 16 * 1024;
  _Float16* sPh = reinterpret_cast<_Float16*>(smem + SM::gfrag);
  _Float16* sPl = QUAD ? sPh + SM::ps : sPh + 8 * SM::ps;
  float* sOut = QUAD ? reinterpret_cast<float*>(sPh) : reinterpret_cast<float*>(sPl + 8 * SM::ps);
  float* sTsv = QUAD ? reinterpret_cast<float*>(sPh + 16 * SM::pcs) : sOut + 8 * SM::os;
  float* sNx = sTsv + 4 * 8 * NQ + (threadIdx.x >> 6) * 256;
  const int tid = threadIdx.x, lane = tid & 63, wv = rfl(tid >> 6);
  const int g = lane >> 4, i = lane & 15, H = lane >> 5, g2 = g & 1;
  const int R = QUAD ? g : H;
  const int gs = QUAD ? 0 : g2;
  const int k = KFULL ? KP : a.k;
  const float gbias = GB ? a.gbias : 0.f, ltgt = GB ? a.loss_tgt_const : 1.f;
  for (int e = tid; e < 4 * 8 * NQ; e += 256) sTsv[e] = 0.f;
  f16x8 gAh[GREG ? 2 : 1][GREG ? 4 : 1], gAl[GREG ? 2 : 1][GREG ? 4 : 1];
  float ginv;
  {
    const int m = lane & 15, kb = lane >> 4;
    float gmax = 0.f;
#pragma unroll
    for (int t = 0; t < 2; t++)
#pragma unroll
      for (int ks = 0; ks < 4; ks++)
#pragma unroll
        for (int e = 0; e < 8; e++) {
          const int r = 32 * wv + 16 * t + m, c = 32 * ks + 8 * kb + e;
          {
            const float gv = a.XtX[(size_t)min(r, k - 1) * k + min(c, k - 1)];
            gmax = fmaxf(gmax, fabsf(gv) * ((r < k && c < k) ? 1.f : 0.f));
          }
        }
    for (int o = 32; o > 0; o >>= 1) gmax = fmaxf(gmax, __shfl_xor(gmax, o));
    const int ge = fp16_scale_exp(gmax);
    const float gs = __uint_as_float((unsigned)ge << 23);
    ginv = __uint_as_float((unsigned)(254 - ge) << 23);
#pragma unroll
    for (int t = 0; t < 2; t++)
#pragma unroll
      for (int ks = 0; ks < 4; ks++) {
        unsigned hi[4], lo[4];
#pragma unroll
        for (int e = 0; e < 8; e += 2) {
          const int r = 32 * wv + 16 * t + m, c = 32 * ks + 8 * kb + e;
          const float g0v = a.XtX[(size_t)min(r, k - 1) * k + min(c, k - 1)];
          const float g0 = g0v * ((r < k && c < k) ? 1.f : 0.f);
          const float g1v = a.XtX[(size_t)min(r, k - 1) * k + min(c + 1, k - 1)];
          const float g1 = g1v * ((r < k && c + 1 < k) ? 1.f : 0.f);
          split_f16(g0 * gs, g1 * gs, hi[e / 2], lo[e / 2]);
        }
        const uint4 h4 = {hi[0], hi[1], hi[2], hi[3]}, l4 = {lo[0], lo[1], lo[2], lo[3]};
        if constexpr (GREG) {
          gAh[t][ks] = __builtin_bit_cast(f16x8, h4);
          gAl[t][ks] = __builtin_bit_cast(f16x8, l4);
        } else {
          *reinterpret_cast<uint4*>(sGf + ((t * 4 + ks) * 2 + 0) * 1024 + lane * 16) = h4;
          *reinterpret_cast<uint4*>(sGf + ((t * 4 + ks) * 2 + 1) * 1024 + lane * 16) = l4;
        }
      }
  }
  __syncthreads();
  float* tacc = sTsv + wv * 8 * NQ + (QUAD ? NQ * g : 2 * NQ * H);
  float* tcur = tacc + 4 * NQ;
  const int lslot = (NQ == 16 && !QUAD) ? i + 16 * g2 : i;
  const bool lgrp = NQ == 16 || g2 == 0;
  const int col = RW * wv + R;
  double wloss = 0.0;
  const int wave_global = blockIdx.x * 4 + wv, total_waves = gridDim.x * 4;
  auto ridx = [&](const int itn) { return (wave_global + itn * total_waves) * RW + R; };
  int row_c = 0, p1_c = 0, p2_c = 0, row_n = 0;
  if (iters > 0 && ridx(0) < n_rows) {
    row_c = rows[ridx(0)];
    p1_c = a.col_ptrs[row_c];
    p2_c = a.col_ptrs[row_c + 1];
  }
  if (iters > 1 && ridx(1) < n_rows) row_n = rows[ridx(1)];

  int idn[GREG ? NQ : 1];
  float cvn[GREG ? NQ : 1], cln = 0.f;
#pragma unroll
  for (int q = 0; q < (GREG ? NQ : 1); q++) {
    idn[q] = 0;
    cvn[q] = 0.f;
  }
  auto request_indices = [&](const bool valid, const int np1, const int ncnt, const int buf) {
    if constexpr (!GREG) {
      const int e = lane & (GL - 1);
      const bool in = valid && e < ncnt;
      float* slot = sNx + buf * 128;
      dma4(in ? static_cast<const void*>(a.row_idx + np1 + e) : static_cast<const void*>(a.zero_row), (unsigned)rfl((int)lds_addr(slot)));
      dma4(in ? static_cast<const void*>(a.vals + np1 + e) : static_cast<const void*>(a.zero_row), (unsigned)rfl((int)lds_addr(slot + 64)));
      return;
    }
#pragma unroll
    for (int q = 0; q < NQ; q++) {
      const int s = 2 * q + g2;
      const int j = (valid && s < ncnt) ? np1 + s : 0;
      idn[q] = a.row_idx[j];
      cvn[q] = a.vals[j];
    }
    cln = a.vals[(valid && lslot < ncnt) ? np1 + lslot : 0];
  };
  auto settle_indices = [&]() {
    if constexpr (!GREG) {
      wait_vm<0>();
      return;
    }
#pragma unroll
    for (int q = 0; q < NQ; q += 8) {
      asm volatile("" : "+v"(idn[q]), "+v"(idn[q + 1]), "+v"(idn[q + 2]), "+v"(idn[q + 3]), "+v"(idn[q + 4]), "+v"(idn[q + 5]), "+v"(idn[q + 6]), "+v"(idn[q + 7]));
      asm volatile("" : "+v"(cvn[q]), "+v"(cvn[q + 1]), "+v"(cvn[q + 2]), "+v"(cvn[q + 3]), "+v"(cvn[q + 4]), "+v"(cvn[q + 5]), "+v"(cvn[q + 6]), "+v"(cvn[q + 7]));
    }
    asm volatile("" : "+v"(cln));
  };
  if constexpr (KFULL) {
    request_indices(iters > 0 && ridx(0) < n_rows, p1_c, p2_c - p1_c, 0);
    settle_indices();
  }

  for (int it = 0; it < iters; ++it) {
    const bool have = ridx(it) < n_rows;
    const int row = have ? row_c : 0, p1 = have ? p1_c : 0, p2 = have ? p2_c : 0;
    {
      int p1_n = 0, p2_n = 0, row_nn = 0;
      if (it + 1 < iters && ridx(it + 1) < n_rows) {
        p1_n = a.col_ptrs[row_n];
        p2_n = a.col_ptrs[row_n + 1];
      }
      if (it + 2 < iters && ridx(it + 2) < n_rows) row_nn = rows[ridx(it + 2)];
      row_c = row_n;
      p1_c = p1_n;
      p2_c = p2_n;
      row_n = row_nn;
    }
    const int cnt = p2 - p1;
    float* yrow = a.Y + (size_t)row * k;
    const bool live = have && (GB || cnt > 0);
    if (have && !live) {
      if constexpr (QUAD) {
#pragma unroll
        for (int b = 0; b < NV; b++) *reinterpret_cast<float4*>(yrow + b * 16 * VW + i * VW) = make_float4(0.f, 0.f, 0.f, 0.f);
      } else {
        for (int e = lane & 31; e < k; e += 32) yrow[e] = 0.f;
      }
    }
    int wcnt = max(__builtin_amdgcn_readlane(cnt, 0), __builtin_amdgcn_readlane(cnt, 32));
    if constexpr (QUAD) wcnt = max(wcnt, max(__builtin_amdgcn_readlane(cnt, 16), __builtin_amdgcn_readlane(cnt, 48)));
    auto blk_on = [&](const int q) { return q < 4 || wcnt > SS * (q & ~3); };

    float x[RPN], r[RPN], p[RPN], ap[RPN];
    auto load_warm_start = [&]() {
#pragma unroll
      for (int b = 0; b < NV; b++) {
        const int off = b * 16 * VW + i * VW;
        float4 pc = make_float4(0.f, 0.f, 0.f, 0.f);
        if (have && off < k) pc = *reinterpret_cast<const float4*>(yrow + off);
        const float* pf = reinterpret_cast<const float*>(&pc);
#pragma unroll
        for (int c = 0; c < VW; c++) x[b * VW + c] = pf[c];
      }
    };
    if constexpr (KFULL) load_warm_start();
    float xt[NQ][RPN], cv[GREG ? NQ : 1];
    const float* nx = sNx + (it & 1) * 128 + (QUAD ? 16 * g : 32 * H);
    {
      int id[NQ];
#pragma unroll
      for (int q = 0; q < NQ; q++) {
        if constexpr (!GREG) {
          id[q] = __float_as_int(QUAD ? nx[q] : nx[2 * q + g2]);
        } else if constexpr (KFULL) {
          id[q] = idn[q];
          cv[q] = cvn[q];
        } else {
          const int s = 2 * q + g2;
          const int j = s < cnt ? p1 + s : 0;
          id[q] = 0;
          cv[q] = 0.f;
          if (blk_on(q)) {
            id[q] = a.row_idx[j];
            cv[q] = a.vals[j];
          }
        }
      }
#pragma unroll
      for (int q = 0; q < NQ; q++) {
        const bool in = SS * q + gs < cnt;
        id[q] = in ? id[q] : 0;
        if constexpr (GREG) cv[q] = in ? cv[q] : 0.f;
      }
#pragma unroll
      for (int q = 0; q < NQ; q++) {
        const bool in = SS * q + gs < cnt;
        const float* src = in ? a.X + (size_t)id[q] * k : a.zero_row;
#pragma unroll
        for (int b = 0; b < NV; b++) {
          const int off = b * 16 * VW + i * VW;
          if constexpr (KFULL) {
            float4 pc = make_float4(0.f, 0.f, 0.f, 0.f);
            if (blk_on(q)) pc = *reinterpret_cast<const float4*>(src + off);
            const float* pf = reinterpret_cast<const float*>(&pc);
#pragma unroll
            for (int c = 0; c < VW; c++) xt[q][b * VW + c] = pf[c];
          } else {
            float4 pc = make_float4(0.f, 0.f, 0.f, 0.f);
            if (blk_on(q)) pc = *reinterpret_cast<const float4*>(src + min(off, k - VW));
            const float* pf = reinterpret_cast<const float*>(&pc);
#pragma unroll
            for (int c = 0; c < VW; c++) xt[q][b * VW + c] = off < k ? pf[c] : 0.f;
          }
        }
      }
    }
    float cl;
    if constexpr (!GREG) cl = nx[64 + lslot];
    else if constexpr (KFULL) cl = (lgrp && lslot < cnt) ? cln : 0.f;
    else cl = (lgrp && lslot < cnt) ? a.vals[p1 + lslot] : 0.f;

    if constexpr (!KFULL) load_warm_start();

    auto sweep = [&](const float(&v)[RPN], const int mode, float(&out)[RPN], float& loss_out) {
      float acc[RPN];
#pragma unroll
      for (int rr = 0; rr < RPN; rr++) acc[rr] = 0.f;
      float vinv = 0.f;
      const int ln = opaque_lane<QUAD>(lane), li = ln & 15, lg = ln >> 4;
      const int lcol = QUAD ? RW * wv + lg : col;
      if (mode != 2) {
        float vmax = 0.f;
#pragma unroll
        for (int rr = 0; rr < RPN; rr++) vmax = fmaxf(vmax, fabsf(v[rr]));
        vmax = row16_max(vmax);
        const int ve = fp16_scale_exp(vmax);
        const float vs = __uint_as_float((unsigned)ve << 23);
        vinv = __uint_as_float((unsigned)(254 - ve) << 23) * (mode == 0 ? -1.f : 1.f);
        if constexpr (QUAD) {
          wave_sync();
#pragma unroll
          for (int b = 0; b < NV; b++) {
            unsigned h0, l0, h1, l1;
            split_f16(v[b * VW] * vs, v[b * VW + 1] * vs, h0, l0);
            split_f16(v[b * VW + 2] * vs, v[b * VW + 3] * vs, h1, l1);
            const int off = lcol * SM::pcs + b * 16 * VW + li * VW;
            *reinterpret_cast<uint2*>(sPh + off) = make_uint2(h0, h1);
            *reinterpret_cast<uint2*>(sPl + off) = make_uint2(l0, l1);
          }
        } else {
          float w4[VW];
#pragma unroll
          for (int c = 0; c < VW; c++) w4[c] = (g2 == 0 ? v[c] : v[VW + c]) * vs;
          unsigned h0, l0, h1, l1;
          split_f16(w4[0], w4[1], h0, l0);
          split_f16(w4[2], w4[3], h1, l1);
          const int off = col * SM::ps + g2 * 16 * VW + i * VW;
          *reinterpret_cast<uint2*>(sPh + off) = make_uint2(h0, h1);
          *reinterpret_cast<uint2*>(sPl + off) = make_uint2(l0, l1);
        }
        __syncthreads();
        f32x4 d0[2], d1[2];
#pragma unroll
        for (int t = 0; t < 2; t++) d0[t] = d1[t] = f32x4{0.f, 0.f, 0.f, 0.f};
        const int nb = QUAD ? li * SM::pcs + 8 * lg : (lane & 7) * SM::ps + 8 * (lane >> 4);
        f16x8 bhs[QUAD ? 4 : 1], bls[QUAD ? 4 : 1];
        if constexpr (QUAD) {
#pragma unroll
          for (int ks = 0; ks < 4; ks++) {
            bhs[ks] = *reinterpret_cast<const f16x8*>(sPh + nb + 32 * ks);
            bls[ks] = *reinterpret_cast<const f16x8*>(sPl + nb + 32 * ks);
          }
          __syncthreads();
        }
#pragma unroll
        for (int ks = 0; ks < 4; ks++) {
          f16x8 bh, bl;
          if constexpr (QUAD) {
            bh = bhs[ks];
            bl = bls[ks];
          } else {
            bh = *reinterpret_cast<const f16x8*>(sPh + nb + 32 * ks);
            bl = *reinterpret_cast<const f16x8*>(sPl + nb + 32 * ks);
          }
#pragma unroll
          for (int t = 0; t < 2; t++) {
            f16x8 ah, al;
            if constexpr (GREG) {
              ah = gAh[t][ks];
              al = gAl[t][ks];
            } else {
              ah = *reinterpret_cast<const f16x8*>(sGf + ((t * 4 + ks) * 2 + 0) * 1024 + (QUAD ? ln : lane) * 16);
              al = *reinterpret_cast<const f16x8*>(sGf + ((t * 4 + ks) * 2 + 1) * 1024 + (QUAD ? ln : lane) * 16);
            }
            d0[t] = __builtin_amdgcn_mfma_f32_16x16x32_f16(ah, bh, d0[t], 0, 0, 0);
            d1[t] = __builtin_amdgcn_mfma_f32_16x16x32_f16(ah, bl, d1[t], 0, 0, 0);
            d1[t] = __builtin_amdgcn_mfma_f32_16x16x32_f16(al, bh, d1[t], 0, 0, 0);
          }
        }
        if (QUAD || (lane & 15) < 8) {
#pragma unroll
          for (int t = 0; t < 2; t++) {
            const f32x4 d = (d0[t] + d1[t]) * ginv;
            float* po = QUAD ? sOut + li * SM::os + 32 * wv + 16 * t + 4 * lg : sOut + (lane & 15) * SM::os + 32 * wv + 16 * t + 4 * (lane >> 4);
            *reinterpret_cast<f32x4*>(po) = d;
          }
        }
      }
      float lacc = 0.f;
      if (mode != 2) {
        float* trec = (mode == 0 ? tacc : tcur) + gs;
#pragma unroll
        for (int q0 = 0; q0 < NQ; q0 += 4) {
          if (blk_on(q0)) {
            float t[4];
            f32x2 s2[4];
#pragma unroll
            for (int u = 0; u < 4; u++) s2[u] = f32x2{0.f, 0.f};
#pragma unroll
            for (int rr = 0; rr < RPN; rr += 2) {
              const f32x2 va = {v[rr], v[rr + 1]};
#pragma unroll
              for (int u = 0; u < 4; u++) {
                const f32x2 xa = {xt[q0 + u][rr], xt[q0 + u][rr + 1]};
                s2[u] = __builtin_elementwise_fma(xa, va, s2[u]);
              }
            }
#pragma unroll
            for (int u = 0; u < 4; u++) t[u] = s2[u].x + s2[u].y;
#pragma unroll
            for (int u = 0; u < 4; u++) t[u] += dpp<0xB1>(t[u]);
#pragma unroll
            for (int u = 0; u < 4; u++) t[u] += dpp<0x4E>(t[u]);
#pragma unroll
            for (int u = 0; u < 4; u++) t[u] += dpp<0x141>(t[u]);
#pragma unroll
            for (int u = 0; u < 4; u++) t[u] += dpp<0x140>(t[u]);
#pragma unroll
            for (int u = 0; u < 4; u++) {
              const int q = q0 + u;
              const float c = GREG ? cv[q] : (QUAD ? nx[64 + q] : nx[64 + 2 * q + g2]);
              trec[SS * q] = t[u];
              const float w = mode == 0 ? c - (c - 1.f) * (GB ? t[u] + gbias : t[u]) : (c - 1.f) * t[u];
#pragma unroll
              for (int rr = 0; rr < RPN; rr++) acc[rr] = fmaf(w, xt[q][rr], acc[rr]);
            }
          }
        }
      } else {
        wave_sync();
        const float t = tacc[lslot];
        const float dd = ltgt - t;
        const float ls = row16_sum((lgrp && lslot < cnt) ? cl * dd * dd : 0.f);
        lacc = QUAD ? ls : pair_sum(ls);
      }
      if (mode != 2) {
        __syncthreads();
        const float f = (QUAD || g2 == 0) ? vinv : 0.f;
#pragma unroll
        for (int b = 0; b < NV; b++) {
          const float* po = QUAD ? sOut + lcol * SM::os + b * 16 * VW + li * VW : sOut + col * SM::os + b * 16 * VW + i * VW;
          const f32x4 o = *reinterpret_cast<const f32x4*>(po);
#pragma unroll
          for (int c = 0; c < VW; c++) acc[b * VW + c] = fmaf(f, o[c], acc[b * VW + c]);
        }
#pragma unroll
        for (int rr = 0; rr < RPN; rr++) out[rr] = QUAD ? acc[rr] : pair_sum(acc[rr]);
        if constexpr (GB) {
          if (mode == 0) {
#pragma unroll
            for (int b = 0; b < NV; b++) {
              const int off = b * 16 * VW + i * VW;
              const float4 pc = *reinterpret_cast<const float4*>(a.rhs_init + min(off, k - VW));
              const float* pf = reinterpret_cast<const float*>(&pc);
#pragma unroll
              for (int c = 0; c < VW; c++) out[b * VW + c] += off < k ? pf[c] : 0.f;
            }
          }
        }
      } else {
        loss_out = lacc;
      }
    };
    auto dot16 = [&](const float(&u)[RPN], const float(&w)[RPN]) {
      float s = 0.f;
#pragma unroll
      for (int rr = 0; rr < RPN; rr++) s = fmaf(u[rr], w[rr], s);
      return row16_sum(s);
    };

    float dummy = 0.f;
    sweep(x, 0, r, dummy);
    if constexpr (KFULL)
      request_indices(it + 1 < iters && ridx(it + 1) < n_rows, p1_c, p2_c - p1_c, (it + 1) & 1);
#pragma unroll
    for (int rr = 0; rr < RPN; rr++) p[rr] = r[rr];
    float rsold = dot16(r, r);
    bool conv = !live;
    for (int itc = 0; itc < a.cg_steps; ++itc) {
      sweep(p, 1, ap, dummy);
      const float pap = dot16(p, ap);
      const float alpha = conv ? 0.f : (float)((double)rsold / (double)pap);
      wave_sync();
      if (lgrp) tacc[lslot] = fmaf(alpha, tcur[lslot], tacc[lslot]);
      wave_sync();
#pragma unroll
      for (int rr = 0; rr < RPN; rr++) {
        x[rr] = fmaf(alpha, p[rr], x[rr]);
        r[rr] = fmaf(-alpha, ap[rr], r[rr]);
      }
      const float rsnew = dot16(r, r);
      if (!conv) {
        if (rsnew < kCgTol) {
          conv = true;
        } else {
          const float beta = (float)((double)rsnew / (double)rsold);
#pragma unroll
          for (int rr = 0; rr < RPN; rr++) p[rr] = fmaf(p[rr], beta, r[rr]);
          rsold = rsnew;
        }
      }
    }
    float rl = 0.f;
    sweep(x, 2, ap, rl);
    if constexpr (KFULL) {
      settle_indices();
    }
    if (live) {
      const float xx = dot16(x, x);
      wloss += (double)rl + a.lambda_loss * (double)xx;
      if (QUAD || g2 == 0) {
#pragma unroll
        for (int b = 0; b < NV; b++) {
          const int off = b * 16 * VW + i * VW;
          if (off < k) {
            float4 pc;
            float* pf = reinterpret_cast<float*>(&pc);
#pragma unroll
            for (int c = 0; c < VW; c++) pf[c] = x[b * VW + c];
            *reinterpret_cast<float4*>(yrow + off) = pc;
          }
        }
      }
    }
  }
  const double other = __shfl(wloss, 32);
  if constexpr (QUAD) {
    const double wsum = (wloss + __shfl(wloss, 16)) + (other + __shfl(wloss, 48));
    if (lane == 0) a.loss_partials[loss_slot0 + (size_t)blockIdx.x * 4 + wv] = wsum;
  } else {
    if (lane == 0) a.loss_partials[loss_slot0 + (size_t)blockIdx.x * 4 + wv] = wloss + other;
  }
}

}

bool cgp_supported(int k, bool implicit) { return implicit && k > 64 && k <= 128 && k % 4 == 0; }
bool cgp_wide_supported(int k, bool implicit, bool gbias) { return implicit && k == 128 && !gbias; }
bool cgp_quad_supported(int k, bool implicit, bool gbias) { return implicit && k == 128 && !gbias; }

hipError_t launch_als_cgp(const AlsArgs& a, const int32_t* rows, int n_rows, CgpForm form, size_t loss_slot0, hipStream_t s,
                          hipEvent_t* ev_slot) {
  const int rpw = cgp_rows_per_wave(form);
  const int grid = cgp_grid(n_rows, rpw);
  if (grid <= 0) return hipSuccess;
  const int iters = cgp_visits(n_rows, rpw);
  const bool gb = a.gbias != 0.f;
  const bool full = !gb && a.k == 128;
  const bool wide = form == kCgpWide, quad = form == kCgpQuad;
  if ((wide || quad) && !full) return hipErrorInvalidValue;
  auto k0 = als_cgp_kernel<false, false>;
  auto k0f = als_cgp_kernel<false, true>;
  auto k1 = als_cgp_kernel<true, false>;
  auto kw = als_cgp_kernel<false, true, 16>;
  auto kq = als_cgp_kernel<false, true, 16, true>;
  const void* fn = quad ? reinterpret_cast<const void*>(kq) : wide ? reinterpret_cast<const void*>(kw)
                        : gb ? reinterpret_cast<const void*>(k1) : (full ? reinterpret_cast<const void*>(k0f) : reinterpret_cast<const void*>(k0));
  const size_t lds = quad ? PairSmem<16, true>::bytes : wide ? PairSmem<16>::bytes : PairSmem<8>::bytes;
  hipError_t err = hipFuncSetAttribute(fn, hipFuncAttributeMaxDynamicSharedMemorySize, (int)lds);
  if (err != hipSuccess) return err;
  prof_note(ev_slot, fn);
  if (quad) hipLaunchKernelGGL(kq, dim3(grid), dim3(256), lds, s, a, rows, n_rows, iters, loss_slot0);
  else if (wide) hipLaunchKernelGGL(kw, dim3(grid), dim3(256), lds, s, a, rows, n_rows, iters, loss_slot0);
  else if (gb) hipLaunchKernelGGL(k1, dim3(grid), dim3(256), lds, s, a, rows, n_rows, iters, loss_slot0);
  else if (full) hipLaunchKernelGGL(k0f, dim3(grid), dim3(256), lds, s, a, rows, n_rows, iters, loss_slot0);
  else hipLaunchKernelGGL(k0, dim3(grid), dim3(256), lds, s, a, rows, n_rows, iters, loss_slot0);
  return hipGetLastError();
}

}
```

rsparse_amd/csrc/wrmf_cgq.hip:

```cpp
#include <algorithm>

#include "wrmf_internal.h"
#include "wrmf_device.h"

namespace rsparse_hip {
namespace {

using namespace dev;

constexpr int kGvFirstMinCapq = 16;
constexpr int kStreamPrefixQ = 4;
constexpr int kIdxPrefetchMaxWpr = 2;

constexpr int kMaxSavedSweeps = 4;

template <int KP>
struct QG {
  static constexpr int RPN = KP / 16;
  static constexpr int VW = RPN >= 4 ? 4 : RPN;
  static constexpr int NV = RPN / VW;
  __device__ static __forceinline__ int elem(int i, int r) { return (r / VW) * (16 * VW) + i * VW + (r % VW); }
};

template <int VW>
// ... 804 lines not shown
          }
          wave_sync();
        }
        if constexpr (CVLDS) {
          if (g == 0) {
#pragma unroll
            for (int b = 0; b < NV; b++) {
              piece_t pc = *x_piece(b);
              float* pf = reinterpret_cast<float*>(&pc);
#pragma unroll
              for (int c = 0; c < VW; c++) pf[c] = fmaf(alpha, p[b * VW + c], pf[c]);
              *x_piece(b) = pc;
            }
          }
        }
#pragma unroll
        for (int rr = 0; rr < RPN; rr++) {
          if constexpr (!CVLDS) x[rr] = fmaf(alpha, p[rr], x[rr]);
          r[rr] = fmaf(-alpha, ap[rr], r[rr]);
        }
        const float rsnew = dot16(r, r);
        if (rsnew < kCgTol) {
          conv = true;
        } else {
          const float beta = (float)((double)rsnew / (double)rsold);
#pragma unroll
          for (int rr = 0; rr < RPN; rr++) p[rr] = fmaf(p[rr], beta, r[rr]);
          rsold = rsnew;
        }
      }
    }
    if constexpr (CVLDS) {
      wave_sync();
#pragma unroll
      for (int b = 0; b < NV; b++) {
        const piece_t pc = *x_piece(b);
        const float* pf = reinterpret_cast<const float*>(&pc);
#pragma unroll
        for (int c = 0; c < VW; c++) x[b * VW + c] = pf[c];
      }
    }
    float rl = 0.f;
    sweep(x, 2, ap, rl, live);
    if constexpr (META_LATE) p1_c = rfl(p1_c), p2_c = rfl(p2_c);
    if constexpr (DMAPF) wait_vm<0>();
    if constexpr (IDXPF && STREAM == 0) {
      asm volatile("" : "+v"(pf_id), "+v"(pf_c));
    }
    if (live && tw == 0) {
      const float xx = dot16(x, x);
      const double wl_row = IMPLICIT ? (double)rl + a.lambda_loss * (double)xx : (double)(rl + lam_use * xx);
      if constexpr (CVLDS) {
        if (lane == 0) *wl_lds += wl_row;
      } else {
        wloss += wl_row;
      }
      if (g == 0) {
#pragma unroll
        for (int b = 0; b < NV; b++) {
          const int off = b * 16 * VW + i * VW;
          if (off < k) {
            piece_t pc;
            float* pf = reinterpret_cast<float*>(&pc);
#pragma unroll
            for (int c = 0; c < VW; c++) pf[c] = x[b * VW + c];
            *reinterpret_cast<piece_t*>(yrow + off) = pc;
          }
        }
      }
    }
  }
  if (lane == 0) a.loss_partials[loss_slot0 + (size_t)blockIdx.x * WAVES + wv] = CVLDS ? *wl_lds : wloss;
}

struct BucketDef { int waves, wpr, capq, stream, max_len; };
constexpr int kNB = 6;
constexpr int kNCfg = 2;
constexpr BucketDef kBuckets[kNCfg][kNB] = {
    {{8, 8, 16, 1, 0x7fffffff}, {8, 8, 16, 0, 512}, {4, 4, 16, 0, 256}, {4, 2, 16, 0, 128}, {4, 1, 16, 0, 64}, {4, 1, 8, 0, 32}},
    {{8, 8, 16, 1, 0x7fffffff}, {4, 4, 32, 0, 512}, {4, 2, 32, 0, 256}, {4, 1, 32, 0, 128}, {4, 1, 16, 0, 64}, {4, 1, 8, 0, 32}},
};
constexpr int cfg_of_kp(int KP) { return KP == 64 ? 1 : 0; }
constexpr int kTeam4Waves = 4, kTeam4Capq = 20;
static_assert(kTeam4Max == kTeam4Waves * kTeam4Capq * 4, "wrmf_internal.h's split and the kernel's capacity");
constexpr int kTeam4WideCapq = 24;
static_assert(kTeam4WideMax == kTeam4Waves * kTeam4WideCapq * 4, "wrmf_schedule.h's split and the wide kernel's capacity");
static_assert(kTeam4Max < kTeam4WideMax && kTeam4WideMax < 512, "the 4-wave launches take bucket 1's rows from its short end");
static_assert(QSmem<128, kTeam4WideCapq, kTeam4Waves, kTeam4Waves, 0, true>::bytes <= 80 * 1024, "the wide team kernel's LDS");
constexpr bool team4_split(int KP, bool GB) { return KP == 128 && !GB; }
int team4_first(const QSchedule& q) { return std::min(std::max(q.team4_first, q.off[1]), q.off[2]); }
int team4_wide_first(const QSchedule& q) { return std::min(std::max(q.team4_wide_first, q.off[1]), team4_first(q)); }

template <int KP, int WAVES, int CAPQ, int WPR, int STREAM, bool IMPLICIT, bool GB, int DMF = 0, bool KFULL = false>
hipError_t launch_bucket(const AlsArgs& a, const int32_t* rows, int n_rows, int grid, size_t slot0, hipStream_t s,
                         hipEvent_t* ev_slot) {
  if (n_rows <= 0) return hipSuccess;
  constexpr bool kDmfGeometry = IMPLICIT && KP == 128 && WAVES == 4 && WPR == 1 && (CAPQ == 8 || CAPQ == 16) && STREAM == 0;
  if constexpr (kDmfGeometry && !DMF) {
    return launch_bucket<KP, WAVES, CAPQ, WPR, STREAM, IMPLICIT, GB, CAPQ == 8 ? 1 : 2>(a, rows, n_rows, grid, slot0, s, ev_slot);
  } else {
    if constexpr (!KFULL && STREAM == 0 && !(DMF == 1 && !GB)) {
      if (a.k == KP)
        return launch_bucket<KP, WAVES, CAPQ, WPR, STREAM, IMPLICIT, GB, DMF, true>(a, rows, n_rows, grid, slot0, s, ev_slot);
    }
    constexpr int TEAMS = WAVES / WPR;
    auto kern = als_cgq_kernel<KP, CAPQ, WAVES, WPR, STREAM, IMPLICIT, DMF, GB, KFULL>;
    const size_t lds = QSmem<KP, CAPQ, WAVES, WPR, STREAM, IMPLICIT, DMF>::bytes;
    hipError_t err = hipFuncSetAttribute(reinterpret_cast<const void*>(kern),
                                         hipFuncAttributeMaxDynamicSharedMemorySize, (int)lds);
    if (err != hipSuccess) return err;
    const int total_teams = grid * TEAMS;
    const int rpt = (n_rows + total_teams - 1) / total_teams;
    prof_note(ev_slot, reinterpret_cast<const void*>(kern));
    hipLaunchKernelGGL(kern, dim3(grid), dim3(WAVES * 64), lds, s, a, rows, n_rows, rpt, slot0);
    return hipGetLastError();
  }
}

struct BucketStreams {
  hipStream_t st[kNB] = {nullptr, nullptr, nullptr, nullptr, nullptr, nullptr};
  hipEvent_t fork = nullptr, fork0 = nullptr;
  hipEvent_t done[kNB] = {nullptr, nullptr, nullptr, nullptr, nullptr, nullptr};
  int device = -1;
  hipError_t ensure() {
    int dev = 0;
    hipError_t err = hipGetDevice(&dev);
    if (err != hipSuccess) return err;
    if (dev == device) return hipSuccess;
    device = dev;
    if ((err = hipEventCreateWithFlags(&fork, hipEventDisableTiming)) != hipSuccess) return err;
    if ((err = hipEventCreateWithFlags(&fork0, hipEventDisableTiming)) != hipSuccess) return err;
    for (int b = 0; b < kNB; b++) {
      if ((err = hipStreamCreateWithFlags(&st[b], hipStreamNonBlocking)) != hipSuccess) return err;
      if ((err = hipEventCreateWithFlags(&done[b], hipEventDisableTiming)) != hipSuccess) return err;
    }
    return hipSuccess;
  }
};
thread_local BucketStreams g_bs;

int g_launch_mode = 2;
int concurrent_buckets() { return g_launch_mode; }

size_t bucket_slots(const QSchedule& q, int b, int k, bool implicit) {
  const int cfg = cfg_of_kp(padded_rank(k));
  const BucketDef d = kBuckets[cfg][b];
  if (d.wpr <= 0) return 0;
  if (d.stream && ne_supported(k)) return (size_t)(q.ne.entries + q.ne.nsplit) + (size_t)(q.mf_n > 0 ? cg_mf_loss_slots(q.mf_n) : 0);
  const int rows = q.off[b + 1] - q.off[b];
  if (b == 1 && padded_rank(k) == 128) {
    const int wide = team4_wide_first(q), split = team4_first(q);
    return (size_t)cgq_bucket_grid(wide - q.off[b], b, cfg) * d.waves + (size_t)cgq_team4_wide_grid(split - wide) * kTeam4Waves +
           (size_t)cgq_team4_grid(q.off[b + 1] - split) * kTeam4Waves;
  }
  if (b == kNB - 1 && rows > 0 && cgp_supported(k, implicit)) {
    const int split = std::min(std::max(q.pair_first, q.off[b]), q.off[b + 1]);
    const size_t main = q.pair_wide ? (size_t)cgp_loss_slots(split - q.off[b], cgp_rows_per_wave(kCgpWide))
                                    : (size_t)cgq_bucket_grid(split - q.off[b], b, cfg) * d.waves;
    return main + (size_t)cgp_loss_slots(q.off[b + 1] - split, cgp_rows_per_wave(q.pair_quad ? kCgpQuad : kCgpPair));
  }
  return (size_t)cgq_bucket_grid(rows, b, cfg) * d.waves;
}

template <int KP, int CFG, bool IMPLICIT, bool GB>
hipError_t launch_all(const AlsArgs& a, const QSchedule& q, hipStream_t s, hipEvent_t* ev) {
  hipError_t err;
  size_t slot = 0;
  const int cmode = ev ? 0 : concurrent_buckets();
  const bool overlap = cmode != 0;
  bool forked = false;
  if (overlap) {
    if ((err = g_bs.ensure()) != hipSuccess) return err;
  }
#define RSP_BUCKET(B)                                                                                       \
  {                                                                                                         \
    constexpr BucketDef D = kBuckets[CFG][B];                                                               \
    if (ev && (err = hipEventRecord(ev[B], s)) != hipSuccess) return err;                                   \
    if constexpr (D.wpr > 0) {                                                                              \
      const int n = q.off[B + 1] - q.off[B];                                                                \
      const int grid = cgq_bucket_grid(n, B, CFG);                                                          \
      if (n > 0) {                                                                                          \
        hipStream_t bs = s;                                                                                 \
        const bool side = overlap && !(cmode == 2 && D.stream);                                             \
        if (side) {                                                                                         \
          if (!forked) {                                                                                    \
            if ((err = hipEventRecord(g_bs.fork, s)) != hipSuccess) return err;                             \
            forked = true;                                                                                  \
          }                                                                                                 \
          bs = g_bs.st[B];                                                                                  \
          if ((err = hipStreamWaitEvent(bs, g_bs.fork, 0)) != hipSuccess) return err;                       \
        }                                                                                                   \
        if (D.stream && ne_supported(a.k)) {                                                                \
           \
           \
           \
           \
          const bool mside = overlap && q.ne.wg > 0 && q.mf_n > 0;                                          \
           \
          if (mside && (err = hipEventRecord(g_bs.fork0, s)) != hipSuccess) return err;                     \
          if (q.ne.wg > 0 &&                                                                                \
              (err = launch_als_ne(a, q, IMPLICIT, a.loss_partials + slot, bs, q.mf_n > 0 ? nullptr : (ev ? ev + B : nullptr))) != hipSuccess) \
            return err;                                                                                     \
          if (q.mf_n > 0) {                                                                                 \
            hipStream_t ms = bs;                                                                            \
            if (mside) {                                                                                    \
              ms = g_bs.st[B];                                                                              \
              if ((err = hipStreamWaitEvent(ms, g_bs.fork0, 0)) != hipSuccess) return err;                  \
            }                                                                                               \
            if ((err = launch_als_cg_mf(a, q.mf_rows, q.mf_n, (int)(slot + (size_t)(q.ne.entries + q.ne.nsplit)), ms, \
                                        ev ? ev + B : nullptr)) != hipSuccess)                              \
              return err;                                                                                   \
            if (mside) {                                                                                    \
              if ((err = hipEventRecord(g_bs.done[B], ms)) != hipSuccess) return err;                       \
              if ((err = hipStreamWaitEvent(s, g_bs.done[B], 0)) != hipSuccess) return err;                 \
            }                                                                                               \
          }                                                                                                 \
        } else if constexpr (D.stream && KP > 32) {        \
          return hipErrorInvalidValue;                                                                      \
        } else if constexpr (B == 1 && team4_split(KP, GB)) {                                              \
           \
           \
          const int first = q.off[B], wide = team4_wide_first(q), split = team4_first(q);                   \
          const int n_main = wide - first, n_w4 = split - wide, n_t4 = q.off[B + 1] - split;                \
          const int g_main = cgq_bucket_grid(n_main, B, CFG), g_w4 = cgq_team4_wide_grid(n_w4);             \
          if ((err = launch_bucket<KP, D.waves, D.capq, D.wpr, D.stream, IMPLICIT, GB>(a, q.order + first, n_main, g_main, slot, \
                                                                                  bs, ev ? ev + B : nullptr)) != hipSuccess) \
            return err;                                                                                     \
          if ((err = launch_bucket<KP, kTeam4Waves, kTeam4WideCapq, kTeam4Waves, 0, IMPLICIT, GB>(          \
                   a, q.order + wide, n_w4, g_w4, slot + (size_t)g_main * D.waves, bs,                      \
                   n_main > 0 ? nullptr : (ev ? ev + B : nullptr))) != hipSuccess)                          \
            return err;                                                                                     \
          if ((err = launch_bucket<KP, kTeam4Waves, kTeam4Capq, kTeam4Waves, 0, IMPLICIT, GB>(              \
                   a, q.order + split, n_t4, cgq_team4_grid(n_t4),                                          \
                   slot + (size_t)g_main * D.waves + (size_t)g_w4 * kTeam4Waves, bs,                        \
                   n_main + n_w4 > 0 ? nullptr : (ev ? ev + B : nullptr))) != hipSuccess)                   \
            return err;                                                                                     \
        } else if (B == kNB - 1 && cgp_supported(a.k, IMPLICIT)) {                    \
           \
                  \
          const int first = q.off[B], split = std::min(std::max(q.pair_first, first), q.off[B + 1]);         \
          const int n_main = split - first, n_pair = q.off[B + 1] - split;                                   \
          size_t main_slots;                                                                                \
          if (q.pair_wide) {                                                                                \
            if ((err = launch_als_cgp(a, q.order + first, n_main, kCgpWide, slot, bs, ev ? ev + B : nullptr)) != hipSuccess) \
              return err;                                                                                   \
            main_slots = (size_t)cgp_loss_slots(n_main, cgp_rows_per_wave(kCgpWide));                       \
          } else {                                                                                          \
            const int g_main = cgq_bucket_grid(n_main, B, CFG);                                             \
            if ((err = launch_bucket<KP, D.waves, D.capq, D.wpr, D.stream, IMPLICIT, GB>(a, q.order + first, n_main, g_main, slot, \
                                                                                    bs, ev ? ev + B : nullptr)) != hipSuccess) \
              return err;                                                                                   \
            main_slots = (size_t)g_main * D.waves;                                                          \
          }                                                                                                 \
          if ((err = launch_als_cgp(a, q.order + split, n_pair, q.pair_quad ? kCgpQuad : kCgpPair, slot + main_slots, bs, \
                                    n_main > 0 ? nullptr : (ev ? ev + B : nullptr))) != hipSuccess)           \
            return err;                                                                                     \
        } else if ((err = launch_bucket<KP, D.waves, D.capq, D.wpr, D.stream, IMPLICIT, GB>(a, q.order + q.off[B], n, grid, slot, \
                                                                                bs, ev ? ev + B : nullptr)) != hipSuccess) \
          return err;                                                                                       \
        if (side) {                                                                                         \
          if ((err = hipEventRecord(g_bs.done[B], bs)) != hipSuccess) return err;                           \
          if ((err = hipStreamWaitEvent(s, g_bs.done[B], 0)) != hipSuccess) return err;                     \
        }                                                                                                   \
      }                                                                                                     \
      slot += bucket_slots(q, B, a.k, IMPLICIT);                                                             \
    }                                                                                                       \
  }
  RSP_BUCKET(0)
  RSP_BUCKET(1)
  RSP_BUCKET(2)
  RSP_BUCKET(3)
  RSP_BUCKET(4)
  RSP_BUCKET(5)
#undef RSP_BUCKET
  if (ev && (err = hipEventRecord(ev[kNB], s)) != hipSuccess) return err;
  return hipSuccess;
}

}

int cgq_num_buckets() { return kNB; }
int cgq_bucket_wpr(int cfg, int b) { return kBuckets[cfg][b].wpr; }
int cgq_bucket_capq(int cfg, int b) { return kBuckets[cfg][b].capq; }
int cgq_bucket_waves(int cfg, int b) { return kBuckets[cfg][b].waves; }
int cgq_bucket_stream(int cfg, int b) { return kBuckets[cfg][b].stream; }

namespace {
int team_grid(int n_rows, int teams, int base) {
  int rows_per_team = base;
  const long spread = (long)teams * 512;
  if ((long)n_rows < spread * rows_per_team) rows_per_team = (int)((n_rows + spread - 1) / spread);
  if (rows_per_team < 1) rows_per_team = 1;
  const long per_wg = (long)teams * rows_per_team;
  long grid = (n_rows + per_wg - 1) / per_wg;
  if (grid < 1) grid = 1;
  return (int)grid;
}
}

int cgq_bucket_grid(int n_rows, int b, int cfg) {
  const BucketDef d = kBuckets[cfg][b];
  if (n_rows <= 0 || d.wpr <= 0) return 0;
  const int base = d.stream ? 16 : (d.wpr == 1 ? 64 : (d.wpr == 2 ? 64 : 32));
  return team_grid(n_rows, d.waves / d.wpr, base);
}

int cgq_team4_grid(int n_rows) { return n_rows <= 0 ? 0 : team_grid(n_rows, 1, 32); }
int cgq_team4_wide_grid(int n_rows) { return cgq_team4_grid(n_rows); }

int cgq_bucket_of(int len, int cfg) {
  int best = 0;
  for (int b = 0; b < kNB; b++)
    if (kBuckets[cfg][b].wpr > 0 && len <= kBuckets[cfg][b].max_len) best = b;
  return best;
}

size_t cgq_loss_slots(const QSchedule& q, int k, bool implicit) {
  size_t n = 0;
  for (int b = 0; b < kNB; b++) n += bucket_slots(q, b, k, implicit);
  return n;
}

int cgq_default_cfg() { return 0; }
void cgq_set_launch_mode(int mode) { g_launch_mode = mode; }

hipError_t launch_als_cgq(const AlsArgs& a, const QSchedule& q, bool implicit, hipStream_t s, hipEvent_t* ev) {
  const int KP = padded_rank(a.k);
#define RSP_DISPATCH(KPV)                                                                                   \
  if (KP == KPV) {                                                                                          \
    if (implicit && a.gbias != 0.f) return launch_all<KPV, cfg_of_kp(KPV), true, true>(a, q, s, ev);        \
    return implicit ? launch_all<KPV, cfg_of_kp(KPV), true, false>(a, q, s, ev)                             \
                    : launch_all<KPV, cfg_of_kp(KPV), false, false>(a, q, s, ev);                           \
  }
  RSP_DISPATCH(32)
  RSP_DISPATCH(64)
  RSP_DISPATCH(128)
#undef RSP_DISPATCH
  return hipErrorInvalidValue;
}

}
```

rsparse_amd/csrc/wrmf_internal.h:

```cpp
#pragma once
#include <hip/hip_runtime.h>
#include <cstdint>
#include <string>

#include "wrmf_schedule.h"

namespace rsparse_hip {

constexpr float kCgTol = 1e-10f;
constexpr double kCgTolD = 1e-10;
constexpr int kScdMaxIter = 10000;
constexpr float kScdTol = 1e-4f;
constexpr double kScdTolD = 1e-4;
constexpr float kNnlsEps = 1e-16f;
constexpr double kNnlsEpsD = 1e-16;

struct NeListSet {
  const int32_t* rows = nullptr;
  const int32_t* ptr = nullptr;
  int wg = 0;
  int entries = 0;
  const int32_t* segs = nullptr;
  int nseg = 0;
  const int32_t* split_rows = nullptr;
  const int32_t* split_ptr = nullptr;
  int nsplit = 0;
};

struct DevCSC {
  int n_rows = 0;
  int n_cols = 0;
  int64_t nnz = 0;
  const int32_t* col_ptrs = nullptr;
  const int32_t* row_idx = nullptr;
  const float* vals = nullptr;
  int n_long = 0;
  int short_max = 0;
  int max_len = 0;
  const int32_t* q_order = nullptr;
  int q_off[7] = {0, 0, 0, 0, 0, 0, 0};
  int q_cfg = 0;
  int q_pair_first = 0;
  int q_team4_first = 0;
  int q_team4_wide_first = 0;
  int64_t q_nnz[6] = {0, 0, 0, 0, 0, 0};
  const int64_t* q_stream_off = nullptr;
  int q_n_chol_long = 0;
  int q_gt32 = 0;
  int q_gt48 = 0;
  int q_lr_first = 0, q_n_lr = 0;
  NeListSet q_ne;
  NeListSet q_ne1;
  int q_n_nec = 0;
  NeListSet q_nec;
  int64_t nnz_long = 0;
  int n_empty = 0;
  mutable bool vals_frozen = false;
  mutable bool vstats_valid = false;
  mutable unsigned* vstats = nullptr;
  mutable hipStream_t vstats_stream = nullptr;
};

struct AlsArgs {
  const int32_t* col_ptrs;
  const int32_t* row_idx;
  const float* vals;
  const float* X;
  float* Y;
  const float* XtX;
  const int32_t* long_rows;
  int n_long;
  int n_cols;
  int k;
  int cg_steps;
  float lambda;
  double lambda_loss;
  int dynamic_lambda;
  double* loss_partials;
  int* fail_counter;
  int* fail_rows;
  int fail_cap;
  const float* zero_row;
  const float* rhs_vals;
  const float* loss_tgt;
  float loss_tgt_const;
  const float* rhs_init;
  float gbias;
  const float* ne_r0;
  const int32_t* ne_r0_slot;
  float* tscr;
  const int64_t* stream_off;
  int64_t stream_nnz;
  const int32_t* chol_long_rows;
  int n_chol_long;
  const int32_t* chol_list;
  int chol_first, chol_n_main, chol_empty_first;
  const int32_t* lr_rows;
  int n_lr;
  int lr_n_gt32, lr_n_gt16;
  int lr_n_gt48;
  float* nnls_lhs;
  const int32_t* nnls_order;
  int lrx;
  unsigned* lr_flags;
  float* lr_M;
  const int32_t* ne_segs;
  float* ne_seg_scratch;
  int* ne_seg_flags;
  int ne_chol;
  int ne_chol_min;
  const unsigned* ne_stats;
  const float* mf_XtX;
  const unsigned* wave_stats;
};

struct QSchedule {
  const int32_t* order;
  int off[7];
  int pair_first;
  int team4_first;
  int team4_wide_first;
  bool pair_wide;
  bool pair_quad = false;
  int cfg;
  NeListSet ne;
  const int32_t* mf_rows = nullptr;
  int mf_n = 0;
};
int cgq_default_cfg();
void cgq_set_launch_mode(int mode);
int cgq_num_buckets();
int cgq_bucket_wpr(int cfg, int b);
int cgq_bucket_capq(int cfg, int b);
int cgq_bucket_waves(int cfg, int b);
int cgq_bucket_stream(int cfg, int b);
int cgq_bucket_grid(int n_rows, int bucket, int cfg);
int cgq_team4_grid(int n_rows);
int cgq_team4_wide_grid(int n_rows);
int cgq_bucket_of(int len, int cfg);
size_t cgq_loss_slots(const QSchedule& q, int k, bool implicit);
bool cgp_supported(int k, bool implicit);
bool cgp_wide_supported(int k, bool implicit, bool gbias);
bool cgp_quad_supported(int k, bool implicit, bool gbias);
enum CgpForm { kCgpPair = 0, kCgpWide = 1, kCgpQuad = 2 };
inline int cgp_rows_per_wave(CgpForm form) { return form == kCgpQuad ? 4 : 2; }
hipError_t launch_als_cgp(const AlsArgs& a, const int32_t* rows, int n_rows, CgpForm form, size_t loss_slot0, hipStream_t s,
                          hipEvent_t* ev_slot);
bool ne_supported(int k);
constexpr int kNeMinLen = 512;
constexpr int kNeSegFloats = 4 * (11 * 16 * 64 + 128 + 2);
hipError_t launch_ne_stats(const float* X, int64_t nx, const float* vals, int64_t nnz, unsigned* stats, hipStream_t s,
                           const float* absmax_hint = nullptr, const unsigned* cached_vstats = nullptr,
                           unsigned* save_vstats = nullptr);
hipError_t launch_als_ne(const AlsArgs& a, const QSchedule& q, bool implicit, double* row_loss, hipStream_t s,
                         hipEvent_t* ev_slot = nullptr);
hipError_t launch_gb_row_terms(const AlsArgs& a, const int32_t* rows, int n, float* out, int32_t* slot_of_row, hipStream_t s);
hipError_t launch_als_cgq(const AlsArgs& a, const QSchedule& q, bool implicit, hipStream_t s, hipEvent_t* ev = nullptr);

constexpr int kWavesPerWG = 4;
constexpr int kRowsPerWGShort = 64;
constexpr int kRowsPerWGLong = 8;

constexpr int kCholMaxGrid = 256 * 96;

size_t cg_loss_slots(int n_cols, int n_long);
size_t chol_loss_slots(int n_cols);

hipError_t launch_als_cg(const AlsArgs& a, bool implicit, hipStream_t s, hipEvent_t* ev = nullptr);
constexpr int kCholLongGrid = 512;
constexpr int kCholLrGrid = 65536;
size_t chol2_loss_slots(int n_cols);
bool chol_lr_supported(const AlsArgs& a, bool implicit);
bool chol_lrx_supported(const AlsArgs& a, bool implicit);
hipError_t launch_als_chol_lrx(const AlsArgs& a, const int32_t* rows, int n_rows, const unsigned* stats, int loss_slot0,
                               hipStream_t s, hipEvent_t* ev_slot);
hipError_t launch_als_chol_lr(const AlsArgs& a, const int32_t* rows, int n_rows, float* M, float* Mt, unsigned* flags,
                              int loss_slot0, hipStream_t s, hipEvent_t* ev_slot = nullptr);
hipError_t launch_als_chol2(const AlsArgs& a, bool implicit, hipStream_t s, hipEvent_t* ev = nullptr);
bool chol_wave_supported(int k);
hipError_t launch_als_chol_wave(const AlsArgs& a, bool implicit, int grid, int loss_slot0, hipStream_t s, hipEvent_t* ev_slot);
constexpr int kCholMfMax = 512;
constexpr int kCholMfGrid = 256 * 32;
bool chol_mf_supported(int k);
int chol_mf_grid(int n_rows);
int chol_mf_loss_slots(int n_rows, bool implicit);
hipError_t launch_als_chol_mf(const AlsArgs& a, bool implicit, const int32_t* rows, int n_rows, int loss_slot0, hipStream_t s,
                              hipEvent_t* ev_slot);
constexpr int kCgMfGrid = 256 * 16;
bool cg_mf_supported(int k, bool implicit);
int cg_mf_grid(int n_rows);
int cg_mf_loss_slots(int n_rows);
hipError_t launch_als_cg_mf(const AlsArgs& a, const int32_t* rows, int n_rows, int loss_slot0, hipStream_t s, hipEvent_t* ev_slot);
hipError_t launch_als_nnls(const AlsArgs& a, bool implicit, hipStream_t s, hipEvent_t* ev = nullptr);
constexpr int kLuGrid = 64;
constexpr int kFailCap = 1 << 16;
hipError_t launch_als_lu_fallback(const AlsArgs& a, bool implicit, size_t loss_slot0, hipStream_t s);
hipError_t launch_fail_roll(int* fails, hipStream_t s);
constexpr int kSumStageBlocks = 256;
hipError_t launch_sum_partials(const double* partials, size_t n, double* out, hipStream_t s, double* tail = nullptr);
hipError_t launch_bias_shift_values(const float* vals, const int32_t* row_idx, const float* X, int k, int bias_row,
                                    int64_t nnz, float* out, hipStream_t s);
hipError_t launch_bias_sweep(const int32_t* p, const int32_t* i, const float* x, const float* other, int n_cols,
                             float lambda, int dynamic_lambda, int non_negative, float* out, hipStream_t s);
hipError_t launch_values_sum(const float* x, int64_t n, double* partials, double* out, hipStream_t s);
hipError_t launch_bias_implicit_terms(const float* vals, const int32_t* row_idx, const float* X, int k, int bias_row,
                                      int64_t nnz, float global_bias, float* rhs_vals, float* loss_tgt, hipStream_t s);
hipError_t launch_bias_rhs_init(const float* X, int k, int off, int k1, int bias_row, float global_bias, int n,
                                float* scratch, float* out, hipStream_t s);
size_t bias_rhs_init_scratch_floats();
hipError_t launch_pad_rows(const float* src, int src_stride, int src_off, int k1, int k1p, int64_t n, float* dst, hipStream_t s);
hipError_t launch_pad_gramian(const float* G, int k1, int k1p, float* Gp, hipStream_t s);
hipError_t launch_bias_implicit_prep(const int32_t* p, const float* x, int n_cols, int n_other, double lambda,
                                     double* means, double* adj, hipStream_t s);
hipError_t launch_bias_implicit_sweep(const int32_t* p, const int32_t* i, const float* x, const float* other, int n_cols,
                                      int n_other, const double* other_sum, const double* means, const double* adj,
                                      int non_negative, double global_bias, float* out, hipStream_t s);
hipError_t launch_values_subtract_mean(float* x, int64_t n, const double* sum, double inv_count, hipStream_t s);

size_t gramian_scratch_floats(int k, int64_t n);
hipError_t launch_gramian(const float* X, int k, int64_t n, float ridge, float* XtX, double* sumsq, float* scratch,
                          hipStream_t s, hipEvent_t* ev = nullptr, unsigned* absmax_bits = nullptr);
hipError_t launch_weighted_sumsq(const float* X, int k, int64_t n, const float* w, double* out,
                                 double* scratch , hipStream_t s);
hipError_t launch_f64_to_f32(const double* in, float* out, size_t n, hipStream_t s);
hipError_t check_row_indices_device(const int32_t* i, int64_t nnz, int n_rows, hipStream_t s, int* bad_index);
hipError_t transpose_csc_device(int n_rows, int n_cols, int64_t nnz, const int32_t* p, const int32_t* i, const float* x,
                                int32_t* pt, int32_t* it, float* xt, hipStream_t s, int* bad_index);
hipError_t launch_f32_to_f64(const float* in, double* out, size_t n, hipStream_t s);

hipError_t launch_top_product(const float* U, const float* V, int n_users, int n_items, int k_rank, int topk,
                              const int32_t* nr_ptr, const int32_t* nr_idx, const int32_t* excl, int n_excl,
                              float glob_mean, int32_t* res, float* scores, hipStream_t s, float* scratch = nullptr);
size_t top_product_f64_scratch_words(int n_users, int kc, int topk);
hipError_t launch_top_product_f64(const float* U32, const float* V32, const double* U64, const double* V64, int n_users,
                                  int n_items, int rank, int topk, int kc, const int32_t* nr_ptr, const int32_t* nr_idx,
                                  const int32_t* excl, int n_excl, double glob_mean, int32_t* res, double* scores, hipStream_t s,
                                  float* scratch, float* split_scratch);
size_t top_product_scratch_entries(int n_users, int n_items, int topk);
size_t top_product_scratch_floats(int n_users, int n_items, int k_rank, int topk);
bool top_product_wants_gbuf(int n_users, int k_rank, int topk);
constexpr int kTopLargeMin = 256;
constexpr int kTopLargeMax = 8192;
size_t top_product_large_ws_floats(int n_users, int n_items, int topk, int kc, int* chunk_users = nullptr);
int top_product_large_kc(int topk, int extra, int n_items);
hipError_t launch_top_product_large(const float* U, const float* V, int n_users, int n_items, int rank, int topk,
                                    const int32_t* nr_ptr, const int32_t* nr_idx, const int32_t* excl, int n_excl, float glob_mean,
                                    int32_t* res, float* scores, hipStream_t s, float* ws);
hipError_t launch_top_product_large_f64(const float* U32, const float* V32, const double* U64, const double* V64, int n_users,
                                        int n_items, int rank, int topk, int kc, const int32_t* nr_ptr, const int32_t* nr_idx,
                                        const int32_t* excl, int n_excl, double glob_mean, int32_t* res, double* scores,
                                        hipStream_t s, float* ws);
hipError_t launch_topl_score(const float* U, const float* V, int nu, int n_items, int rank, unsigned* keys, size_t ld, hipStream_t s);
hipError_t launch_topl_mask(unsigned* keys, size_t ld, int n_items, int nu, const int32_t* nr_ptr, const int32_t* nr_idx,
                            const int32_t* excl, int n_excl, hipStream_t s);

size_t held_out_ranks_ws_floats(int n_users, int n_items, int max_chunk_users, int* chunk_users = nullptr);
hipError_t launch_held_out_ranks(const float* U, const float* V, int n_users, int n_items, int rank, const int32_t* nr_ptr,
                                 const int32_t* nr_idx, const int32_t* excl, int n_excl, const int32_t* act_ptr,
                                 const int32_t* act_idx, int max_chunk_users, int32_t* above, int32_t* tied, int32_t* n_adm,
                                 hipStream_t s, float* ws);
hipError_t launch_rank_summary(int n_users, const int32_t* act_ptr, const double* act_x, const int32_t* above, const int32_t* tied,
                               const int32_t* n_adm, double* mpr, double* auc, double* mrr, double* sums, hipStream_t s);

hipError_t launch_ranking_metrics(const int32_t* pred, int n_users, int k, const int32_t* P, const int32_t* J, const double* X,
                                  double* ap_out, double* ndcg_out, int* long_buf, hipStream_t s);

constexpr int kHitMaxCutoffs = 16;
hipError_t launch_hit_metrics(const int32_t* pred, int n_users, int k, const int32_t* P, const int32_t* J, const int32_t* cutoffs,
                              int n_cutoffs, int32_t* hits, int32_t* first, double* precision, double* recall, double* hit,
                              double* mrr, int32_t* first_seen, int n_items, hipStream_t s);

hipError_t launch_list_metrics(const int32_t* pred, int n_users, int k, const int32_t* cutoffs, int n_cutoffs,
                               const int32_t* item_count, const int64_t* item_info, int n_items, int32_t* valid, int64_t* count_sum,
                               int64_t* info_sum, double* popularity, double* novelty, int32_t* exposure, hipStream_t s);

hipError_t launch_item_inv_norms(const void* V, bool f64, int n_items, int64_t ld, int c0, int r, double* inv, hipStream_t s);
hipError_t launch_list_diversity(const int32_t* pred, int n_users, int k, const int32_t* cutoffs, int n_cutoffs, const void* V,
                                 bool f64, int n_items, int64_t ld, int c0, int r, const double* inv, int32_t* counted,
                                 double* diversity, hipStream_t s);

hipError_t launch_mmr_rerank(const int32_t* lists, const double* scores, int n_users, int n_pool, int k, double theta, const void* V,
                             bool f64, int n_items, int64_t ld, int c0, int r, const double* inv, int32_t* items, double* picked,
                             int32_t* positions, double* objective, hipStream_t s);

template <class T>
hipError_t launch_score_pairs(const T* U, const T* V, int n_rows, int n_cols, int r, const int32_t* P, const int32_t* J, double add,
                              double* scores, hipStream_t s);
hipError_t launch_score_error_sums(const double* scores, const double* actual, const int32_t* P, int n_rows, double* sse,
                                   double* sae, hipStream_t s);

size_t top_candidates_ws_bytes(int n_users, int64_t nnz);
template <class T>
hipError_t launch_top_candidates(const T* U, const T* V, int n_users, int n_items, int rank, int topk, const int32_t* cand_p,
                                 const int32_t* cand_j, int32_t p0, int64_t nnz, const int32_t* nr_ptr, const int32_t* nr_idx,
                                 const int32_t* excl, int n_excl, double glob_mean, int32_t* res, double* scores, hipStream_t s,
                                 void* ws);

// ... 143 lines not shown
```

rsparse_amd/csrc/wrmf_schedule.cpp:

```cpp
#include "wrmf_schedule.h"

#include <algorithm>
#include <functional>
#include <queue>
#include <utility>

namespace rsparse_hip {

namespace {
int ne_slots(int cus) { return 2 * std::max(cus, 1); }
}

int cgp_grid(int n_rows, int rows_per_wave) {
  if (n_rows <= 0) return 0;
  const long sets = ((long)n_rows + rows_per_wave - 1) / rows_per_wave;
  long per_wave = 32;
  const long spread = 4L * 512;
  if (sets < spread * per_wave) per_wave = (sets + spread - 1) / spread;
  if (per_wave < 1) per_wave = 1;
  return (int)((sets + 4 * per_wave - 1) / (4 * per_wave));
}
int cgp_visits(int n_rows, int rows_per_wave) {
  const long grid = cgp_grid(n_rows, rows_per_wave);
  if (grid <= 0) return 0;
  const long sets = ((long)n_rows + rows_per_wave - 1) / rows_per_wave;
  return (int)((sets + grid * 4 - 1) / (grid * 4));
}
int64_t cgp_loss_slots(int n_rows, int rows_per_wave) { return (int64_t)cgp_grid(n_rows, rows_per_wave) * 4; }

NeCut ne_cut(const int32_t* order, const int32_t* col_ptrs, int n_prefix, int64_t fixed, int cus) {
  NeCut c;
  if (n_prefix <= 0) return c;
  auto len_of = [&](int r) { return (int64_t)(col_ptrs[order[r] + 1] - col_ptrs[order[r]]); };
  auto steps_of = [](int64_t len) { return (len + 15) / 16; };
  const int n_slots = ne_slots(cus);
  int64_t total = 0;
  for (int r = 0; r < n_prefix; r++) total += steps_of(len_of(r)) + fixed;
  const int64_t share = std::max<int64_t>(1, total / n_slots);
  c.items.reserve((size_t)n_prefix + 64);
  int n_seg = 0;
  for (int r = 0; r < n_prefix; r++) {
    const int64_t len = len_of(r);
    const int64_t st = steps_of(len);
    int parts = 1;
    if (n_slots >= 8 && 2 * (st + fixed) > share)
      parts = (int)std::min<int64_t>(std::min<int64_t>(kNeMaxSeg, st / 64), (4 * st + share - 1) / share);
    if (parts < 2 || n_seg + parts > kNeMaxSegTotal) {
      c.items.push_back({st + fixed, order[r]});
      continue;
    }
    const int64_t per = (st + parts - 1) / parts;
    const int slot = n_seg;
    const int made = (int)((st + per - 1) / per);
    int idx = 0;
    for (int64_t s0 = 0; s0 < st; s0 += per, idx++) {
      const int64_t n0 = s0 * 16, n1 = std::min(len, (s0 + per) * 16);
      c.segs.insert(c.segs.end(), {order[r], (int32_t)n0, (int32_t)(n1 - n0), idx, made, slot});
      c.items.push_back({steps_of(n1 - n0) + fixed, -(int32_t)(n_seg + 1)});
      n_seg++;
    }
    c.split_rows.push_back(-(int32_t)(slot + 1));
  }
  if (n_seg > 0)
    for (size_t i = 0; i <= c.split_rows.size(); i++) c.split_ptr.push_back((int32_t)i);
  std::stable_sort(c.items.begin(), c.items.end(), [](const NeCut::Item& x, const NeCut::Item& y) { return x.cost > y.cost; });
  return c;
}

NeDeal ne_deal(const NeCut& cut, int n_prefix, int cus, bool fine) {
  NeDeal d;
  const size_t n_items = cut.items.size();
  if (!n_items) return d;
  const int n_slots = ne_slots(cus);
  int n_wg = fine ? std::max(n_slots, std::min(n_prefix / 8, 256 * std::max(cus, 1))) : n_slots;
  n_wg = (int)std::min<size_t>((size_t)n_wg, n_items);
  std::vector<int> owner(n_items);
  d.ptr.assign((size_t)n_wg + 1, 0);
  std::priority_queue<std::pair<int64_t, int>, std::vector<std::pair<int64_t, int>>, std::greater<>> heap;
  for (int w = 0; w < n_wg; w++) heap.push({0, w});
  for (size_t e = 0; e < n_items; e++) {
    auto top = heap.top();
    heap.pop();
    owner[e] = top.second;
    d.ptr[(size_t)top.second + 1]++;
    heap.push({top.first + cut.items[e].cost, top.second});
  }
  for (int w = 0; w < n_wg; w++) d.ptr[(size_t)w + 1] += d.ptr[(size_t)w];
  d.rows.resize(n_items);
  std::vector<int32_t> fill(d.ptr.begin(), d.ptr.end() - 1);
  for (size_t e = 0; e < n_items; e++) d.rows[(size_t)fill[(size_t)owner[e]]++] = cut.items[e].entry;
  return d;
}

bool plan_schedule(const int32_t* col_ptrs, int n_cols, int cus, int (*bucket_of)(int len), SchedulePlan& out) {
  out = SchedulePlan();
  const int n = n_cols;
  int max_len = 0;
  for (int i = 0; i < n; i++) {
    const int len = col_ptrs[i + 1] - col_ptrs[i];
    if (len < 0) return false;
    max_len = std::max(max_len, len);
  }
  out.max_len = max_len;
  if (n <= 0) {
    out.nec_is_ne = true;
    return true;
  }
  std::vector<int64_t> start((size_t)max_len + 2, 0);
  for (int i = 0; i < n; i++) start[(size_t)(max_len - (col_ptrs[i + 1] - col_ptrs[i])) + 1]++;
  int cnt_b[6] = {0, 0, 0, 0, 0, 0};
  for (int len = max_len; len >= 0; len--) {
    const int cnt = (int)start[(size_t)(max_len - len) + 1];
    if (!cnt) continue;
    if (len > kTileNnz) { out.n_long += cnt; out.nnz_long += (int64_t)len * cnt; }
    if (len == 0) out.n_empty += cnt;
    if (len > kCholLongLen) out.n_chol_long += cnt;
    if (len > kCgMfMax) out.n_nec += cnt;
    if (len > 16) out.pair_first += cnt;
    if (len > kTeam4Max) out.team4_first += cnt;
    if (len > kTeam4WideMax) out.team4_wide_first += cnt;
    if (len > 32) out.gt32 += cnt;
    if (len > 48) out.gt48 += cnt;
    if (len > kCholLrMax) out.lr_first += cnt;
    else if (len >= 1) out.n_lr += cnt;
    const int b = bucket_of(len);
    cnt_b[b] += cnt;
    out.nnz[b] += (int64_t)len * cnt;
  }
  for (int b = 0; b < 6; b++) out.off[b + 1] = out.off[b] + cnt_b[b];
  for (size_t b = 1; b < start.size(); b++) start[b] += start[b - 1];
  out.order.resize((size_t)n);
  for (int i = 0; i < n; i++) out.order[(size_t)start[(size_t)(max_len - (col_ptrs[i + 1] - col_ptrs[i]))]++] = i;
  const int n_stream = out.off[1];
  if (n_stream > 0) {
    out.stream_off.assign((size_t)n_stream + 1, 0);
    for (int r = 0; r < n_stream; r++) {
      const int row = out.order[(size_t)r];
      out.stream_off[(size_t)r + 1] = out.stream_off[(size_t)r] + (col_ptrs[row + 1] - col_ptrs[row]);
    }
    out.cut = ne_cut(out.order.data(), col_ptrs, n_stream, 12, cus);
    out.fine = ne_deal(out.cut, n_stream, cus, true);
    out.coarse = ne_deal(out.cut, n_stream, cus, false);
  }
  out.nec_is_ne = out.n_nec == n_stream;
  if (!out.nec_is_ne) {
    out.cut_nec = ne_cut(out.order.data(), col_ptrs, out.n_nec, 12, cus);
    out.nec = ne_deal(out.cut_nec, out.n_nec, cus, true);
  }
  return true;
}

}
```

rsparse_amd/csrc/wrmf_schedule.h:

```cpp
#pragma once
#include <cstdint>
#include <vector>

namespace rsparse_hip {

constexpr int kTileNnz = 32;
constexpr int kTeam4Max = 320;
constexpr int kTeam4WideMax = 384;
constexpr int kCholLrMax = 64;
constexpr int kCholLongLen = 4096;
constexpr int kCgMfMax = 16384;
constexpr int kNeMaxSeg = 16;
constexpr int kNeMaxSegTotal = 1024;

int cgp_grid(int n_rows, int rows_per_wave = 2);
int cgp_visits(int n_rows, int rows_per_wave = 2);
int64_t cgp_loss_slots(int n_rows, int rows_per_wave = 2);

struct NeCut {
  struct Item { int64_t cost; int32_t entry; };
  std::vector<Item> items;
  std::vector<int32_t> segs;
  std::vector<int32_t> split_rows;
  std::vector<int32_t> split_ptr;
  int nseg() const { return (int)(segs.size() / 6); }
};
struct NeDeal {
  std::vector<int32_t> rows, ptr;
  int wg() const { return ptr.empty() ? 0 : (int)ptr.size() - 1; }
};

NeCut ne_cut(const int32_t* order, const int32_t* col_ptrs, int n_prefix, int64_t fixed, int cus);
NeDeal ne_deal(const NeCut& cut, int n_prefix, int cus, bool fine);

struct SchedulePlan {
  int max_len = 0;
  int n_long = 0;
  int64_t nnz_long = 0;
  int n_empty = 0;
  std::vector<int32_t> order;
  int off[7] = {0, 0, 0, 0, 0, 0, 0};
  int64_t nnz[6] = {0, 0, 0, 0, 0, 0};
  int pair_first = 0;
  int team4_first = 0;
  int team4_wide_first = 0;
  int gt32 = 0, gt48 = 0;
  int lr_first = 0, n_lr = 0;
  int n_chol_long = 0;
  int n_nec = 0;
  std::vector<int64_t> stream_off;
  NeCut cut, cut_nec;
  NeDeal fine, coarse, nec;
  bool nec_is_ne = false;
};

bool plan_schedule(const int32_t* col_ptrs, int n_cols, int cus, int (*bucket_of)(int len), SchedulePlan& out);

}
```

Measured before the change: 8.907 iterations/s.

## Route rows with 33-40 non-zeros to a new 40-slot pair CG kernel

Adds a 'mid' variant of the pair conjugate-gradient kernel (NQ=20 quads, 40 slots) and sends rows of the second-to-last bucket with at most 40 non-zeros to it instead of the generic bucket kernel. The indices and values of slots beyond 32 are fetched by an extra DMA into a widened LDS staging area, and the fp16 split Gram product is folded into a single MFMA accumulator. The aim is to give these mid-length rows the cheaper fused-pair path that rows of 32 or fewer non-zeros already use. In exchange the kernel grows more complex, LDS use per workgroup rises, and there is one more launch plus a split of the bucket.

```diff
diff --git a/include/rsparse_wrmf_hip.h b/include/rsparse_wrmf_hip.h
--- a/include/rsparse_wrmf_hip.h
+++ b/include/rsparse_wrmf_hip.h
@@ -88,6 +88,7 @@
 int rsparse_hip_csc_freeze_values(rsparse_hip_csc* m, int frozen);
 
 int rsparse_hip_csc_info(const rsparse_hip_csc* m, int64_t info_out[40]);
+int rsparse_hip_cgp_mid_max(void);
 
 int rsparse_hip_gramian_device(const float* d_X, int rank, int64_t n, double lambda,
                                float* d_XtX_out, double* d_sumsq_out, void* stream);
diff --git a/rsparse_amd/_lib.py b/rsparse_amd/_lib.py
--- a/rsparse_amd/_lib.py
+++ b/rsparse_amd/_lib.py
@@ -34,6 +34,7 @@
     "rsparse_hip_gramian_absmax_device": (_c_int, [_vp, _c_int, _c_i64, _c_dbl, _vp, _vp, _vp, _vp]),
     "rsparse_hip_csc_destroy": (_c_int, [_vp]),
     "rsparse_hip_csc_info": (_c_int, [_vp, ctypes.POINTER(_c_i64)]),
+    "rsparse_hip_cgp_mid_max": (_c_int, []),
     "rsparse_hip_csc_freeze_values": (_c_int, [_vp, _c_int]),
     "rsparse_hip_als_implicit_bias_device": (_c_int, [_vp, _vp, _vp, _vp, _c_int, _c_dbl, _c_uint, _c_int, _vp, _vp]),
     "rsparse_hip_als_implicit_global_bias_device": (_c_int, [_vp, _vp, _vp, _vp, _c_int, _c_dbl, _c_uint, _c_uint, _c_int,
diff --git a/rsparse_amd/build.py b/rsparse_amd/build.py
--- a/rsparse_amd/build.py
+++ b/rsparse_amd/build.py
@@ -19,7 +19,7 @@
 AUDITED = {"wrmf_chol_mf.hip", "wrmf_cg_mf.hip"}
 REG_LIMIT = {"wrmf_cg_mf.hip": 512}
 NO_SPILL = {"wrmf_cgq.hip": ("14als_cgq_kernelILi128ELi24ELi4ELi4E",),
-            "wrmf_cgp.hip": ("14als_cgp_kernelILb0ELb1ELi16ELb1E",),
+            "wrmf_cgp.hip": ("14als_cgp_kernelILb0ELb1ELi16ELb1E", "14als_cgp_kernelILb0ELb1ELi20ELb0E"),
             "wrmf_explain.hip": ("14explain_kernelIfLi128E",),
             "wrmf_sample.hip": ("13sample_kernelILi64E", "13sample_kernelILi256E"),
             "wrmf_sample_weighted.hip": ("22sample_weighted_kernelILi64E", "22sample_weighted_kernelILi256E"),
diff --git a/rsparse_amd/csrc/wrmf_capi.cpp b/rsparse_amd/csrc/wrmf_capi.cpp
--- a/rsparse_amd/csrc/wrmf_capi.cpp
+++ b/rsparse_amd/csrc/wrmf_capi.cpp
@@ -158,6 +158,7 @@
   for (int b = 0; b < 7; b++) d.q_off[b] = plan.off[b];
   for (int b = 0; b < 6; b++) d.q_nnz[b] = plan.nnz[b];
   d.q_pair_first = plan.pair_first; d.q_team4_first = plan.team4_first;
+  d.q_pair_mid_first = plan.pair_mid_first;
   d.q_team4_wide_first = plan.team4_wide_first;
   d.q_gt32 = plan.gt32; d.q_gt48 = plan.gt48; d.q_lr_first = plan.lr_first; d.q_n_lr = plan.n_lr;
   d.q_n_chol_long = plan.n_chol_long; d.q_n_nec = plan.n_nec;
@@ -311,6 +312,8 @@
   qs.team4_wide_first = (implicit && bias && bias->gbias != 0.f) ? d.q_off[2] : d.q_team4_wide_first;
   qs.pair_wide = cgp_wide_supported(rank, implicit, implicit && bias && bias->gbias != 0.f);
   qs.pair_quad = cgp_quad_supported(rank, implicit, implicit && bias && bias->gbias != 0.f);
+  qs.pair_mid_first = d.q_pair_mid_first;
+  qs.pair_mid = cgp_mid_supported(rank, implicit, implicit && bias && bias->gbias != 0.f);
   const bool cg_mf = cgq && implicit && !bias && cg_mf_supported(rank, implicit) && d.q_order && d.q_off[1] > d.q_n_nec;
   if (cg_mf) {
     qs.mf_rows = d.q_order + d.q_n_nec;
@@ -786,6 +789,8 @@
   info_out[6] = m->d.n_empty; info_out[7] = m->d.short_max;
   return RSPARSE_HIP_OK;
 }
+
+int rsparse_hip_cgp_mid_max(void) { return kPairMidMax; }
 
 int rsparse_hip_set_launch_mode(int mode) {
   if (mode < 0 || mode > 2) return fail(RSPARSE_HIP_ERR_INVALID, "launch mode must be 0, 1 or 2");
diff --git a/rsparse_amd/csrc/wrmf_cgp.hip b/rsparse_amd/csrc/wrmf_cgp.hip
--- a/rsparse_amd/csrc/wrmf_cgp.hip
+++ b/rsparse_amd/csrc/wrmf_cgp.hip
@@ -7,27 +7,33 @@
 using namespace dev;
 
 constexpr int kPairMaxSweeps = 4;
+constexpr int kPairMidQuads = 20;
+static_assert(kPairMidMax == 2 * kPairMidQuads, "wrmf_schedule.h's split and the kernel's capacity");
 
 template <int NQ, bool QUAD = false>
 struct PairSmem {
   static constexpr int KP = 128, ps = KP + 8, os = QUAD ? KP + 8 : KP + 4;
   static constexpr int cols = QUAD ? 16 : 8;
   static constexpr int pcs = QUAD ? 2 * ps : ps;
-  static constexpr size_t gfrag = NQ == 16 ? (size_t)4 * 16 * 1024 : 0;
-  static constexpr size_t nxt = NQ == 16 ? (size_t)4 * 2 * 2 * 64 * 4 : 0;
+  static constexpr size_t gfrag = NQ >= 16 ? (size_t)4 * 16 * 1024 : 0;
+  static constexpr int es = NQ > 16 ? 4 * NQ : 64;
+  static constexpr size_t nxt = NQ >= 16 ? (size_t)4 * 2 * 2 * es * 4 : 0;
   static constexpr size_t pub = (size_t)2 * cols * ps * 2, out = (size_t)cols * os * 4;
   static_assert(!QUAD || (pub == out && (size_t)pcs * 2 == (size_t)os * 4), "QUAD: one column, one stretch of LDS");
   static constexpr size_t bytes = gfrag + (QUAD ? pub : pub + out) + (size_t)4 * 8 * NQ * 4 + nxt + 16;
 };
-static_assert(PairSmem<16>::bytes <= 81920 && PairSmem<16, true>::bytes <= 81920, "two workgroups per CU");
+static_assert(PairSmem<16>::bytes <= 81920 && PairSmem<16, true>::bytes <= 81920 && PairSmem<kPairMidQuads>::bytes <= 81920,
+              "two workgroups per CU");
 
 template <bool GB, bool KFULL = false, int NQ = 8, bool QUAD = false>
 __global__ __launch_bounds__(256, 2) void als_cgp_kernel(AlsArgs a, const int32_t* __restrict__ rows, int n_rows, int iters,
                                                         size_t loss_slot0) {
   constexpr int KP = 128, RPN = 8, VW = 4, NV = 2;
-  static_assert(NQ == 8 || (NQ == 16 && KFULL && !GB), "the 32-slot kernel: rank 128, no global bias");
+  static_assert(NQ == 8 || (NQ >= 16 && NQ % 4 == 0 && NQ <= 24 && KFULL && !GB), "the 32-slot and longer kernels: rank 128, no global bias");
   static_assert(!QUAD || NQ == 16, "four rows per wave: 16 slots per group, G in LDS");
   constexpr bool GREG = NQ == 8;
+  constexpr bool MID = NQ > 16;
+  constexpr int ES = PairSmem<NQ, QUAD>::es, TL = 2 * NQ - 32;
   constexpr int RW = QUAD ? 4 : 2, GL = 64 / RW;
   constexpr int SS = QUAD ? 1 : 2;
   using SM = PairSmem<NQ, QUAD>;
@@ -37,7 +43,7 @@
   _Float16* sPl = QUAD ? sPh + SM::ps : sPh + 8 * SM::ps;
   float* sOut = QUAD ? reinterpret_cast<float*>(sPh) : reinterpret_cast<float*>(sPl + 8 * SM::ps);
   float* sTsv = QUAD ? reinterpret_cast<float*>(sPh + 16 * SM::pcs) : sOut + 8 * SM::os;
-  float* sNx = sTsv + 4 * 8 * NQ + (threadIdx.x >> 6) * 256;
+  float* sNx = sTsv + 4 * 8 * NQ + (threadIdx.x >> 6) * (4 * ES);
   const int tid = threadIdx.x, lane = tid & 63, wv = rfl(tid >> 6);
   const int g = lane >> 4, i = lane & 15, H = lane >> 5, g2 = g & 1;
   const int R = QUAD ? g : H;
@@ -93,8 +99,8 @@
   __syncthreads();
   float* tacc = sTsv + wv * 8 * NQ + (QUAD ? NQ * g : 2 * NQ * H);
   float* tcur = tacc + 4 * NQ;
-  const int lslot = (NQ == 16 && !QUAD) ? i + 16 * g2 : i;
-  const bool lgrp = NQ == 16 || g2 == 0;
+  const int lslot = (NQ >= 16 && !QUAD) ? i + 16 * g2 : i;
+  const bool lgrp = NQ >= 16 || g2 == 0;
   const int col = RW * wv + R;
   double wloss = 0.0;
   const int wave_global = blockIdx.x * 4 + wv, total_waves = gridDim.x * 4;
@@ -116,11 +122,24 @@
   }
   auto request_indices = [&](const bool valid, const int np1, const int ncnt, const int buf) {
     if constexpr (!GREG) {
-      const int e = lane & (GL - 1);
+      const int rl = opaque_lane<MID>(lane);
+      const int e = (MID ? rl : lane) & (GL - 1);
       const bool in = valid && e < ncnt;
-      float* slot = sNx + buf * 128;
+      float* slot = sNx + buf * (2 * ES);
       dma4(in ? static_cast<const void*>(a.row_idx + np1 + e) : static_cast<const void*>(a.zero_row), (unsigned)rfl((int)lds_addr(slot)));
-      dma4(in ? static_cast<const void*>(a.vals + np1 + e) : static_cast<const void*>(a.zero_row), (unsigned)rfl((int)lds_addr(slot + 64)));
+      dma4(in ? static_cast<const void*>(a.vals + np1 + e) : static_cast<const void*>(a.zero_row), (unsigned)rfl((int)lds_addr(slot + ES)));
+      if constexpr (MID) {
+        const int p1a = __builtin_amdgcn_readlane(np1, 0), p1b = __builtin_amdgcn_readlane(np1, 32);
+        const int cna = __builtin_amdgcn_readlane(valid ? ncnt : 0, 0), cnb = __builtin_amdgcn_readlane(valid ? ncnt : 0, 32);
+        const bool up = rl >= TL;
+        const int tp1 = up ? p1b : p1a, tcnt = up ? cnb : cna;
+        const int te = 32 + (up ? rl - TL : rl);
+        const bool tin = te < tcnt;
+        if (rl < 2 * TL) {
+          dma4(tin ? static_cast<const void*>(a.row_idx + tp1 + te) : static_cast<const void*>(a.zero_row), (unsigned)rfl((int)lds_addr(slot + 64)));
+          dma4(tin ? static_cast<const void*>(a.vals + tp1 + te) : static_cast<const void*>(a.zero_row), (unsigned)rfl((int)lds_addr(slot + ES + 64)));
+        }
+      }
       return;
     }
 #pragma unroll
@@ -193,13 +212,14 @@
     };
     if constexpr (KFULL) load_warm_start();
     float xt[NQ][RPN], cv[GREG ? NQ : 1];
-    const float* nx = sNx + (it & 1) * 128 + (QUAD ? 16 * g : 32 * H);
+    const float* nx = sNx + (it & 1) * (2 * ES) + (QUAD ? 16 * g : 32 * H);
+    auto nxs = [&](const int s) { return (MID && s >= 32) ? s + 32 - 32 * H + TL * H : s; };
     {
       int id[NQ];
 #pragma unroll
       for (int q = 0; q < NQ; q++) {
         if constexpr (!GREG) {
-          id[q] = __float_as_int(QUAD ? nx[q] : nx[2 * q + g2]);
+          id[q] = __float_as_int(QUAD ? nx[q] : nx[nxs(2 * q + g2)]);
         } else if constexpr (KFULL) {
           id[q] = idn[q];
           cv[q] = cvn[q];
@@ -244,7 +264,8 @@
       }
     }
     float cl;
-    if constexpr (!GREG) cl = nx[64 + lslot];
+    if constexpr (MID) cl = 0.f;
+    else if constexpr (!GREG) cl = nx[64 + lslot];
     else if constexpr (KFULL) cl = (lgrp && lslot < cnt) ? cln : 0.f;
     else cl = (lgrp && lslot < cnt) ? a.vals[p1 + lslot] : 0.f;
 
@@ -255,8 +276,8 @@
 #pragma unroll
       for (int rr = 0; rr < RPN; rr++) acc[rr] = 0.f;
       float vinv = 0.f;
-      const int ln = opaque_lane<QUAD>(lane), li = ln & 15, lg = ln >> 4;
-      const int lcol = QUAD ? RW * wv + lg : col;
+      const int ln = opaque_lane<QUAD || MID>(lane), li = ln & 15, lg = ln >> 4;
+      const int lcol = QUAD ? RW * wv + lg : (MID ? RW * wv + (ln >> 5) : col);
       if (mode != 2) {
         float vmax = 0.f;
 #pragma unroll
@@ -283,7 +304,7 @@
           unsigned h0, l0, h1, l1;
           split_f16(w4[0], w4[1], h0, l0);
           split_f16(w4[2], w4[3], h1, l1);
-          const int off = col * SM::ps + g2 * 16 * VW + i * VW;
+          const int off = MID ? lcol * SM::ps + (lg & 1) * 16 * VW + li * VW : col * SM::ps + g2 * 16 * VW + i * VW;
           *reinterpret_cast<uint2*>(sPh + off) = make_uint2(h0, h1);
           *reinterpret_cast<uint2*>(sPl + off) = make_uint2(l0, l1);
         }
@@ -291,7 +312,7 @@
         f32x4 d0[2], d1[2];
 #pragma unroll
         for (int t = 0; t < 2; t++) d0[t] = d1[t] = f32x4{0.f, 0.f, 0.f, 0.f};
-        const int nb = QUAD ? li * SM::pcs + 8 * lg : (lane & 7) * SM::ps + 8 * (lane >> 4);
+        const int nb = QUAD ? li * SM::pcs + 8 * lg : (MID ? (ln & 7) * SM::ps + 8 * lg : (lane & 7) * SM::ps + 8 * (lane >> 4));
         f16x8 bhs[QUAD ? 4 : 1], bls[QUAD ? 4 : 1];
         if constexpr (QUAD) {
 #pragma unroll
@@ -318,19 +339,25 @@
               ah = gAh[t][ks];
               al = gAl[t][ks];
             } else {
-              ah = *reinterpret_cast<const f16x8*>(sGf + ((t * 4 + ks) * 2 + 0) * 1024 + (QUAD ? ln : lane) * 16);
-              al = *reinterpret_cast<const f16x8*>(sGf + ((t * 4 + ks) * 2 + 1) * 1024 + (QUAD ? ln : lane) * 16);
+              ah = *reinterpret_cast<const f16x8*>(sGf + ((t * 4 + ks) * 2 + 0) * 1024 + ((QUAD || MID) ? ln : lane) * 16);
+              al = *reinterpret_cast<const f16x8*>(sGf + ((t * 4 + ks) * 2 + 1) * 1024 + ((QUAD || MID) ? ln : lane) * 16);
             }
-            d0[t] = __builtin_amdgcn_mfma_f32_16x16x32_f16(ah, bh, d0[t], 0, 0, 0);
-            d1[t] = __builtin_amdgcn_mfma_f32_16x16x32_f16(ah, bl, d1[t], 0, 0, 0);
-            d1[t] = __builtin_amdgcn_mfma_f32_16x16x32_f16(al, bh, d1[t], 0, 0, 0);
-          }
-        }
-        if (QUAD || (lane & 15) < 8) {
+            if constexpr (MID) {
+              d0[t] = __builtin_amdgcn_mfma_f32_16x16x32_f16(ah, bl, d0[t], 0, 0, 0);
+              d0[t] = __builtin_amdgcn_mfma_f32_16x16x32_f16(al, bh, d0[t], 0, 0, 0);
+              d0[t] = __builtin_amdgcn_mfma_f32_16x16x32_f16(ah, bh, d0[t], 0, 0, 0);
+            } else {
+              d0[t] = __builtin_amdgcn_mfma_f32_16x16x32_f16(ah, bh, d0[t], 0, 0, 0);
+              d1[t] = __builtin_amdgcn_mfma_f32_16x16x32_f16(ah, bl, d1[t], 0, 0, 0);
+              d1[t] = __builtin_amdgcn_mfma_f32_16x16x32_f16(al, bh, d1[t], 0, 0, 0);
+            }
+          }
+        }
+        if (QUAD || ((MID ? li : (lane & 15)) < 8)) {
 #pragma unroll
           for (int t = 0; t < 2; t++) {
-            const f32x4 d = (d0[t] + d1[t]) * ginv;
-            float* po = QUAD ? sOut + li * SM::os + 32 * wv + 16 * t + 4 * lg : sOut + (lane & 15) * SM::os + 32 * wv + 16 * t + 4 * (lane >> 4);
+            const f32x4 d = (MID ? d0[t] : d0[t] + d1[t]) * ginv;
+            float* po = (QUAD || MID) ? sOut + li * SM::os + 32 * wv + 16 * t + 4 * lg : sOut + (lane & 15) * SM::os + 32 * wv + 16 * t + 4 * (lane >> 4);
             *reinterpret_cast<f32x4*>(po) = d;
           }
         }
@@ -367,7 +394,7 @@
 #pragma unroll
             for (int u = 0; u < 4; u++) {
               const int q = q0 + u;
-              const float c = GREG ? cv[q] : (QUAD ? nx[64 + q] : nx[64 + 2 * q + g2]);
+              const float c = GREG ? cv[q] : (QUAD ? nx[64 + q] : nx[ES + nxs(2 * q + g2)]);
               trec[SS * q] = t[u];
               const float w = mode == 0 ? c - (c - 1.f) * (GB ? t[u] + gbias : t[u]) : (c - 1.f) * t[u];
 #pragma unroll
@@ -379,7 +406,13 @@
         wave_sync();
         const float t = tacc[lslot];
         const float dd = ltgt - t;
-        const float ls = row16_sum((lgrp && lslot < cnt) ? cl * dd * dd : 0.f);
+        float lv = (lgrp && lslot < cnt) ? (MID ? nx[ES + lslot] : cl) * dd * dd : 0.f;
+        if constexpr (MID) {
+          const int s2 = 32 + (i & (TL - 1));
+          const float d2 = ltgt - tacc[s2];
+          lv += (g2 == 0 && i < TL && s2 < cnt) ? nx[ES + nxs(s2)] * d2 * d2 : 0.f;
+        }
+        const float ls = row16_sum(lv);
         lacc = QUAD ? ls : pair_sum(ls);
       }
       if (mode != 2) {
@@ -387,7 +420,7 @@
         const float f = (QUAD || g2 == 0) ? vinv : 0.f;
 #pragma unroll
         for (int b = 0; b < NV; b++) {
-          const float* po = QUAD ? sOut + lcol * SM::os + b * 16 * VW + li * VW : sOut + col * SM::os + b * 16 * VW + i * VW;
+          const float* po = (QUAD || MID) ? sOut + lcol * SM::os + b * 16 * VW + li * VW : sOut + col * SM::os + b * 16 * VW + i * VW;
           const f32x4 o = *reinterpret_cast<const f32x4*>(po);
 #pragma unroll
           for (int c = 0; c < VW; c++) acc[b * VW + c] = fmaf(f, o[c], acc[b * VW + c]);
@@ -431,6 +464,9 @@
       const float alpha = conv ? 0.f : (float)((double)rsold / (double)pap);
       wave_sync();
       if (lgrp) tacc[lslot] = fmaf(alpha, tcur[lslot], tacc[lslot]);
+      if constexpr (MID) {
+        if (g2 == 0 && i < TL) tacc[32 + i] = fmaf(alpha, tcur[32 + i], tacc[32 + i]);
+      }
       wave_sync();
 #pragma unroll
       for (int rr = 0; rr < RPN; rr++) {
@@ -486,6 +522,7 @@
 bool cgp_supported(int k, bool implicit) { return implicit && k > 64 && k <= 128 && k % 4 == 0; }
 bool cgp_wide_supported(int k, bool implicit, bool gbias) { return implicit && k == 128 && !gbias; }
 bool cgp_quad_supported(int k, bool implicit, bool gbias) { return implicit && k == 128 && !gbias; }
+bool cgp_mid_supported(int k, bool implicit, bool gbias) { return implicit && k == 128 && !gbias; }
 
 hipError_t launch_als_cgp(const AlsArgs& a, const int32_t* rows, int n_rows, CgpForm form, size_t loss_slot0, hipStream_t s,
                           hipEvent_t* ev_slot) {
@@ -495,20 +532,22 @@
   const int iters = cgp_visits(n_rows, rpw);
   const bool gb = a.gbias != 0.f;
   const bool full = !gb && a.k == 128;
-  const bool wide = form == kCgpWide, quad = form == kCgpQuad;
-  if ((wide || quad) && !full) return hipErrorInvalidValue;
+  const bool wide = form == kCgpWide, quad = form == kCgpQuad, mid = form == kCgpMid;
+  if ((wide || quad || mid) && !full) return hipErrorInvalidValue;
   auto k0 = als_cgp_kernel<false, false>;
   auto k0f = als_cgp_kernel<false, true>;
   auto k1 = als_cgp_kernel<true, false>;
   auto kw = als_cgp_kernel<false, true, 16>;
   auto kq = als_cgp_kernel<false, true, 16, true>;
-  const void* fn = quad ? reinterpret_cast<const void*>(kq) : wide ? reinterpret_cast<const void*>(kw)
+  auto km = als_cgp_kernel<false, true, kPairMidQuads>;
+  const void* fn = mid ? reinterpret_cast<const void*>(km) : quad ? reinterpret_cast<const void*>(kq) : wide ? reinterpret_cast<const void*>(kw)
                         : gb ? reinterpret_cast<const void*>(k1) : (full ? reinterpret_cast<const void*>(k0f) : reinterpret_cast<const void*>(k0));
-  const size_t lds = quad ? PairSmem<16, true>::bytes : wide ? PairSmem<16>::bytes : PairSmem<8>::bytes;
+  const size_t lds = mid ? PairSmem<kPairMidQuads>::bytes : quad ? PairSmem<16, true>::bytes : wide ? PairSmem<16>::bytes : PairSmem<8>::bytes;
   hipError_t err = hipFuncSetAttribute(fn, hipFuncAttributeMaxDynamicSharedMemorySize, (int)lds);
   if (err != hipSuccess) return err;
   prof_note(ev_slot, fn);
-  if (quad) hipLaunchKernelGGL(kq, dim3(grid), dim3(256), lds, s, a, rows, n_rows, iters, loss_slot0);
+  if (mid) hipLaunchKernelGGL(km, dim3(grid), dim3(256), lds, s, a, rows, n_rows, iters, loss_slot0);
+  else if (quad) hipLaunchKernelGGL(kq, dim3(grid), dim3(256), lds, s, a, rows, n_rows, iters, loss_slot0);
   else if (wide) hipLaunchKernelGGL(kw, dim3(grid), dim3(256), lds, s, a, rows, n_rows, iters, loss_slot0);
   else if (gb) hipLaunchKernelGGL(k1, dim3(grid), dim3(256), lds, s, a, rows, n_rows, iters, loss_slot0);
   else if (full) hipLaunchKernelGGL(k0f, dim3(grid), dim3(256), lds, s, a, rows, n_rows, iters, loss_slot0);
diff --git a/rsparse_amd/csrc/wrmf_cgq.hip b/rsparse_amd/csrc/wrmf_cgq.hip
--- a/rsparse_amd/csrc/wrmf_cgq.hip
+++ b/rsparse_amd/csrc/wrmf_cgq.hip
@@ -980,6 +980,11 @@
     const int wide = team4_wide_first(q), split = team4_first(q);
     return (size_t)cgq_bucket_grid(wide - q.off[b], b, cfg) * d.waves + (size_t)cgq_team4_wide_grid(split - wide) * kTeam4Waves +
            (size_t)cgq_team4_grid(q.off[b + 1] - split) * kTeam4Waves;
+  }
+  if (b == kNB - 2 && rows > 0 && q.pair_mid) {
+    const int split = pair_mid_split(q.off[b], q.off[b + 1], q.pair_mid_first);
+    return (size_t)cgq_bucket_grid(split - q.off[b], b, cfg) * d.waves +
+           (size_t)cgp_loss_slots(q.off[b + 1] - split, cgp_rows_per_wave(kCgpMid));
   }
   if (b == kNB - 1 && rows > 0 && cgp_supported(k, implicit)) {
     const int split = std::min(std::max(q.pair_first, q.off[b]), q.off[b + 1]);
@@ -1063,6 +1068,18 @@
                    slot + (size_t)g_main * D.waves + (size_t)g_w4 * kTeam4Waves, bs,                        \
                    n_main + n_w4 > 0 ? nullptr : (ev ? ev + B : nullptr))) != hipSuccess)                   \
             return err;                                                                                     \
+        } else if (B == kNB - 2 && q.pair_mid) {                                                            \
+           \
+                \
+          const int first = q.off[B], split = pair_mid_split(first, q.off[B + 1], q.pair_mid_first);        \
+          const int n_main = split - first, n_mid = q.off[B + 1] - split;                                   \
+          const int g_main = cgq_bucket_grid(n_main, B, CFG);                                               \
+          if ((err = launch_bucket<KP, D.waves, D.capq, D.wpr, D.stream, IMPLICIT, GB>(a, q.order + first, n_main, g_main, slot, \
+                                                                                  bs, ev ? ev + B : nullptr)) != hipSuccess) \
+            return err;                                                                                     \
+          if ((err = launch_als_cgp(a, q.order + split, n_mid, kCgpMid, slot + (size_t)g_main * D.waves, bs, \
+                                    n_main > 0 ? nullptr : (ev ? ev + B : nullptr))) != hipSuccess)           \
+            return err;                                                                                     \
         } else if (B == kNB - 1 && cgp_supported(a.k, IMPLICIT)) {                    \
            \
                   \
diff --git a/rsparse_amd/csrc/wrmf_internal.h b/rsparse_amd/csrc/wrmf_internal.h
--- a/rsparse_amd/csrc/wrmf_internal.h
+++ b/rsparse_amd/csrc/wrmf_internal.h
@@ -41,6 +41,7 @@
   int q_off[7] = {0, 0, 0, 0, 0, 0, 0};
   int q_cfg = 0;
   int q_pair_first = 0;
+  int q_pair_mid_first = 0;
   int q_team4_first = 0;
   int q_team4_wide_first = 0;
   int64_t q_nnz[6] = {0, 0, 0, 0, 0, 0};
@@ -122,6 +123,8 @@
   int team4_wide_first;
   bool pair_wide;
   bool pair_quad = false;
+  int pair_mid_first = 0;
+  bool pair_mid = false;
   int cfg;
   NeListSet ne;
   const int32_t* mf_rows = nullptr;
@@ -142,7 +145,8 @@
 bool cgp_supported(int k, bool implicit);
 bool cgp_wide_supported(int k, bool implicit, bool gbias);
 bool cgp_quad_supported(int k, bool implicit, bool gbias);
-enum CgpForm { kCgpPair = 0, kCgpWide = 1, kCgpQuad = 2 };
+bool cgp_mid_supported(int k, bool implicit, bool gbias);
+enum CgpForm { kCgpPair = 0, kCgpWide = 1, kCgpQuad = 2, kCgpMid = 3 };
 inline int cgp_rows_per_wave(CgpForm form) { return form == kCgpQuad ? 4 : 2; }
 hipError_t launch_als_cgp(const AlsArgs& a, const int32_t* rows, int n_rows, CgpForm form, size_t loss_slot0, hipStream_t s,
                           hipEvent_t* ev_slot);
diff --git a/rsparse_amd/csrc/wrmf_schedule.cpp b/rsparse_amd/csrc/wrmf_schedule.cpp
--- a/rsparse_amd/csrc/wrmf_schedule.cpp
+++ b/rsparse_amd/csrc/wrmf_schedule.cpp
@@ -27,6 +27,7 @@
   return (int)((sets + grid * 4 - 1) / (grid * 4));
 }
 int64_t cgp_loss_slots(int n_rows, int rows_per_wave) { return (int64_t)cgp_grid(n_rows, rows_per_wave) * 4; }
+int pair_mid_split(int first, int end, int pair_mid_first) { return std::min(std::max(pair_mid_first, first), end); }
 
 NeCut ne_cut(const int32_t* order, const int32_t* col_ptrs, int n_prefix, int64_t fixed, int cus) {
   NeCut c;
@@ -117,6 +118,7 @@
     if (len > kCholLongLen) out.n_chol_long += cnt;
     if (len > kCgMfMax) out.n_nec += cnt;
     if (len > 16) out.pair_first += cnt;
+    if (len > kPairMidMax) out.pair_mid_first += cnt;
     if (len > kTeam4Max) out.team4_first += cnt;
     if (len > kTeam4WideMax) out.team4_wide_first += cnt;
     if (len > 32) out.gt32 += cnt;
diff --git a/rsparse_amd/csrc/wrmf_schedule.h b/rsparse_amd/csrc/wrmf_schedule.h
--- a/rsparse_amd/csrc/wrmf_schedule.h
+++ b/rsparse_amd/csrc/wrmf_schedule.h
@@ -7,6 +7,7 @@
 constexpr int kTileNnz = 32;
 constexpr int kTeam4Max = 320;
 constexpr int kTeam4WideMax = 384;
+constexpr int kPairMidMax = 40;
 constexpr int kCholLrMax = 64;
 constexpr int kCholLongLen = 4096;
 constexpr int kCgMfMax = 16384;
@@ -16,6 +17,7 @@
 int cgp_grid(int n_rows, int rows_per_wave = 2);
 int cgp_visits(int n_rows, int rows_per_wave = 2);
 int64_t cgp_loss_slots(int n_rows, int rows_per_wave = 2);
+int pair_mid_split(int first, int end, int pair_mid_first);
 
 struct NeCut {
   struct Item { int64_t cost; int32_t entry; };
@@ -42,6 +44,7 @@
   int off[7] = {0, 0, 0, 0, 0, 0, 0};
   int64_t nnz[6] = {0, 0, 0, 0, 0, 0};
   int pair_first = 0;
+  int pair_mid_first = 0;
   int team4_first = 0;
   int team4_wide_first = 0;
   int gt32 = 0, gt48 = 0;
```

Result: no change. 8.939 iterations/s (median of 6 runs) (+0.4%).
